# LeeYN-43/Clover

Measured on AMD Instinct MI355X. Metric: video-text pairs/sec (8f x 224^2, 32-tok), full pre-training step, higher is better.
Workload: dtype f16; 1 GPU; VideoSwin-T + BERT-base + 3-layer fusion, MLM + tri-modal exclusive InfoNCE + rank losses, 8f x 224^2, 32-tok; per_gpu_batch=8, global_batch=8, parallelism=dp1

## Files before the change

### clover_amd/_lib.py

```python
import ctypes as C
import os

_HERE = os.path.dirname(os.path.abspath(__file__))
HALF_F16 = os.environ.get('CLOVER_HALF', 'f16').lower() in ('f16', 'fp16', 'float16', 'half')
LIB_PATH = os.environ.get('CLOVER_LIB_PATH') or os.path.join(_HERE, 'libclover_hip_f16.so' if HALF_F16 else 'libclover_hip.so')


_scale_env = os.environ.get('CLOVER_LOSS_SCALE', '1024' if HALF_F16 else '1')
LOSS_SCALE_SPEC = 'dynamic' if _scale_env.strip().lower() == 'dynamic' else float(_scale_env)
LOSS_SCALE = (1024.0 if HALF_F16 else 1.0) if LOSS_SCALE_SPEC == 'dynamic' else LOSS_SCALE_SPEC


def half_dtype():
    import torch
    return torch.float16 if HALF_F16 else torch.bfloat16

ABI_VERSION = 18

ERRORS = {-1: 'CLV_ERR_ARG (bad argument)', -2: 'CLV_ERR_UNSUPPORTED (shape not supported by the kernels)',
          -3: 'CLV_ERR_LAUNCH (HIP launch failed)'}


class ClvAttnGeom(C.Structure):
    _fields_ = [(n, C.c_int32) for n in
                ('mode', 'groups', 'N', 'nH', 'hd', 'D', 'H', 'W', 'wd', 'wh', 'ww', 'sd', 'sh', 'sw',
                 'ldq', 'ldk', 'ldv', 'ldo', 'bwd', 'bwh', 'bww')] + [('scale', C.c_float), ('dropout_p', C.c_float),
                                                                      ('dbias_index', C.c_void_p), ('work', C.c_void_p)]


_p, _i32, _i64, _f = C.c_void_p, C.c_int32, C.c_int64, C.c_float


class ClvFoldEntry(C.Structure):
    _fields_ = [('partial', _p), ('dw', _p), ('db', _p), ('nk', _i64), ('e2', _i64), ('splits', _i32),
                ('sg_shift', _i32), ('block_begin', _i32), ('overwrite', _i32)]


FOLD_MAX = 64


class ClvWgradEntry(C.Structure):
    _fields_ = [('dy', _p), ('x', _p), ('work', _p), ('dw', _p), ('db', _p), ('M', _i64), ('work_floats', _i64),
                ('N', _i32), ('K', _i32),
                ('ldy', _i32), ('ldx', _i32), ('want_bias', _i32), ('splits', _i32), ('overwrite', _i32), ('pad', _i32)]


WGRAD_GROUP_MAX = 80


class ClvDbiasGather(C.Structure):
    _fields_ = [('partial', _p), ('dtable', _p), ('index', _p), ('split_stride', _i64), ('nkt', _i32), ('nH', _i32),
                ('N', _i32), ('nsplit', _i32), ('slot0', _i32), ('nslots', _i32), ('block_begin', _i32), ('pad', _i32)]


DBIAS_GATHER_MAX = 32


class ClvLnReduceEntry(C.Structure):
    _fields_ = [('partial', _p), ('dgamma', _p), ('dbeta', _p), ('nblk', _i32), ('C', _i32), ('block_begin', _i32),
                ('pad', _i32)]


LN_REDUCE_MAX = 64


class ClvLnExtra(C.Structure):
    _fields_ = [('xscale', _p), ('rows_per_sample', _i32), ('drop_p', _f), ('seed', _p), ('dy2', _p), ('dres', _p),
                ('x_is_sum', _i32), ('gather_c', _i32), ('gather_h2', _i32), ('gather_w2', _i32), ('no_reduce', _i32),
                ('q8', _p), ('qscale', _p)]


SIGNATURES = {
    'clv_abi_version': (C.c_int, []),
    'clv_half_type': (C.c_int, []),
    'clv_attn_fwd': (C.c_int, [_p] * 9 + [C.POINTER(ClvAttnGeom), _p]),
    'clv_attn_seq_work_bytes': (C.c_int64, [C.POINTER(ClvAttnGeom)]),
    'clv_attn_seq_max_keys': (C.c_int, []),
    'clv_attn_seq_parts': (C.c_int, [C.POINTER(ClvAttnGeom)]),
    'clv_attn_bwd_work_bytes': (C.c_int64, [C.POINTER(ClvAttnGeom)]),
    'clv_attn_bwd_one_kernel': (C.c_int, [C.POINTER(ClvAttnGeom)]),
    'clv_attn_dbias_index_count': (C.c_int64, [C.POINTER(ClvAttnGeom)]),
    'clv_attn_dbias_index': (C.c_int, [C.POINTER(ClvAttnGeom), _p, _p]),
    'clv_attn_dbias_gather_entry': (C.c_int, [C.POINTER(ClvAttnGeom), _p, _p, C.POINTER(ClvDbiasGather)]),
    'clv_attn_dbias_partial_bytes': (C.c_int64, [_p]),
    'clv_attn_dbias_gather_batch': (C.c_int, [C.POINTER(ClvDbiasGather), _i32, _p]),
    'clv_attn_bwd': (C.c_int, [_p] * 16 + [_i32, C.POINTER(ClvAttnGeom), _p]),
    'clv_softmax_rows_fwd': (C.c_int, [_p] * 5 + [_i64, _i32, _i32, _i32, _f, _f, _p]),
    'clv_softmax_rows_bwd': (C.c_int, [_p] * 4 + [_i64, _i32, _i32, _f, _f, _p]),
    'clv_layernorm_fwd': (C.c_int, [_p] * 8 + [_i64, _i32, _f, _i32, C.POINTER(ClvLnExtra), _p]),
    'clv_layernorm_bwd_blocks': (C.c_int, [_i64, _i32]),
    'clv_layernorm_bwd': (C.c_int, [_p] * 11 + [_i64, _i32, _i32, C.POINTER(ClvLnExtra), _p]),
    'clv_ln_fold_fwd': (C.c_int, [_p] * 6 + [_i32, _i32, _p]),
    'clv_ln_fold_bwd': (C.c_int, [_p] * 9 + [_i32, _i32, _p]),
    'clv_batchnorm1d_fwd': (C.c_int, [_p] * 8 + [_i32, _i32, _f, _f, _i32, _p]),
    'clv_batchnorm1d_bwd': (C.c_int, [_p] * 8 + [_i32, _i32, _i32, _p]),
    'clv_gelu_fwd': (C.c_int, [_p, _p, _i64, _i32, _p]),
    'clv_gelu_bwd': (C.c_int, [_p, _p, _p, _i64, _i32, _p]),
    'clv_patch_embed_fwd': (C.c_int, [_p] * 12 + [_i32] * 7 + [_f, _p]),
    'clv_patch_embed_fwd_fp8': (C.c_int, [_p] * 13 + [_i32] * 7 + [_f, _p]),
    'clv_patch_embed_blend_bwd': (C.c_int, [_p] * 5 + [_i32] * 7 + [_p]),
    'clv_im2col_patches': (C.c_int, [_p, _p, _i32, _i32, _i32, _i32, _p]),
    'clv_linear_wgrad_work_floats': (C.c_int64, [_i64, _i32, _i32]),
    'clv_linear_wgrad': (C.c_int, [_p] * 5 + [_i64, _i32, _i32, _i32, _i32, _p, _p, _i32, _p]),
    'clv_rowgemm_supported': (C.c_int, [_i32, _i32, _i32]),
    'clv_rowgemm': (C.c_int, [_p] * 11 + [_i64, _i32, _i32, _i32, _i32, _i32, _i32, _f, _p]),
    'clv_rowgemm_xs': (C.c_int, [_p] * 11 + [_i64, _i32, _i32, _i32, _i32, _i32, _i32, _f, _p, _i32, _p]),
    'clv_mlp_fused_supported': (C.c_int, [_i32, _i32]),
    'clv_mlp_fused_fwd': (C.c_int, [_p] * 10 + [_i64, _i32, _i32, _f, _p, _i32, _p]),
    'clv_mlp_fused_bwd': (C.c_int, [_p] * 13 + [_i64, _i32, _i32, _p, _i32, _p]),
    'clv_colsum': (C.c_int, [_p, _p, _i64, _i32, _i32, _p]),
    'clv_focal_ce_fwd': (C.c_int, [_p, _i32, _p, _p, _p, _p, _p, _i64, _i32, _f, _p]),
    'clv_focal_ce_bwd': (C.c_int, [_p, _i32, _p, _p, _p, _p, _p, _p, _i64, _i32, _f, _p]),
    'clv_focal_ce_fwd_ld': (C.c_int, [_p, _i32, _p, _p, _p, _p, _p, _i64, _i32, _i64, _f, _p]),
    'clv_focal_ce_bwd_ld': (C.c_int, [_p, _i32, _p, _p, _p, _p, _p, _p, _i64, _i32, _i64, _f, _p]),
    'clv_infonce_work_floats': (C.c_int64, [_i32, _i32]),
    'clv_infonce_fwd': (C.c_int, [_p] * 6 + [_i32, _i32, _i32, _f, _f, _p]),
    'clv_infonce_bwd': (C.c_int, [_p] * 10 + [_i32, _i32, _i32, _f, _f, _p]),
    'clv_infonce_pair_fwd': (C.c_int, [_p] * 4 + [_i32, _i32, _i32, _f, _f, _p]),
    'clv_infonce_pair_bwd': (C.c_int, [_p] * 4 + [_i32, _i32, _i32, _f, _f, _p]),
    'clv_normsoftmax_work_floats': (C.c_int64, [_i32, _i32]),
    'clv_normsoftmax_fwd': (C.c_int, [_p] * 5 + [_i32, _i32, _f, _f, _p]),
    'clv_normsoftmax_bwd': (C.c_int, [_p] * 6 + [_i32, _i32, _f, _p]),
    'clv_infonce_large_min_g': (C.c_int32, []),
    'clv_infonce_fwd_large': (C.c_int, [_p] * 6 + [_i32, _i32, _i32, _f, _f, _p]),
    'clv_infonce_bwd_large': (C.c_int, [_p] * 10 + [_i32, _i32, _i32, _f, _f, _p]),
    'clv_infonce_pair_fwd_large': (C.c_int, [_p] * 4 + [_i32, _i32, _i32, _f, _f, _p]),
    'clv_infonce_pair_bwd_large': (C.c_int, [_p] * 4 + [_i32, _i32, _i32, _f, _f, _p]),
    'clv_normsoftmax_fwd_large': (C.c_int, [_p] * 5 + [_i32, _i32, _f, _f, _p]),
    'clv_normsoftmax_bwd_large': (C.c_int, [_p] * 6 + [_i32, _i32, _f, _p]),
    'clv_sumsq': (C.c_int, [_p, _p, _i64, _p]),
    'clv_adamw_step': (C.c_int, [_p] * 6 + [_i64] + [_f] * 9 + [_p]),
    'clv_gemm_nt_supported': (C.c_int, [_i64, _i32, _i32]),
    'clv_gemm_nt': (C.c_int, [_p] * 6 + [_i64, _i32, _i32, _i64, _i64, _i64, _i32, _p]),
    'clv_gemm_nt_work_bytes': (C.c_int64, [_i64, _i32, _i32]),
    'clv_gemm_nt_ex': (C.c_int, [_p] * 6 + [_i64, _i32, _i32, _i64, _i64, _i64, _i32, _p, _i64, _p]),
    'clv_transpose_batch': (C.c_int, [_p, _p, _p, _i32, _i32, _p]),
    'clv_layernorm_bwd_needs_reduce': (C.c_int, [_i64, _i32]),
    'clv_ln_reduce_batch': (C.c_int, [_p, _i32, _p]),
    'clv_linear_wgrad_in_place': (C.c_int, [C.c_int64, C.c_int32, C.c_int32]),
    'clv_linear_wgrad_class': (C.c_int, [C.c_int64, C.c_int32, C.c_int32]),
    'clv_linear_wgrad_batch_plan': (C.c_int, [_p, _i32]),
    'clv_linear_wgrad_batch': (C.c_int, [_p, _i32, _p]),
    'clv_linear_wgrad_batch_ss': (C.c_int, [_p, _i32, _p, _p]),
    'clv_linear_wgrad_splits': (C.c_int, [_i64, _i32, _i32]),
    'clv_wgrad_fold_batch': (C.c_int, [_p, _i32, _p]),
    'clv_wgrad_fold_batch_ss': (C.c_int, [_p, _i32, _p, _p]),
    'clv_optim_prep_slots': (C.c_int, [_p, _p, _p] + [_f] * 4 + [_p]),
    'clv_sumsq_ranges': (C.c_int, [_p, _p, _i32, _p, _p]),
    'clv_optim_prep': (C.c_int, [_p, _p] + [_f] * 4 + [_p]),
    'clv_adamw_step_dev': (C.c_int, [_p] * 6 + [_i64] + [_f] * 5 + [_p]),
    'clv_ema_update': (C.c_int, [_p, _i32, _i32, C.c_double, _p]),
    'clv_ema_swap': (C.c_int, [_p, _i32, _i32, _p]),
    'clv_grad_report': (C.c_int, [_p, _i32, _p, _i32, _i32, _p, _p, _i32, _p]),
    'clv_quant_fp8_rows': (C.c_int, [_p, _p, _p, _i64, _i32, _i64, _i64, _p]),
    'clv_gemm_nt_fp8_supported': (C.c_int, [_i64, _i32, _i32]),
    'clv_gemm_nt_fp8': (C.c_int, [_p] * 7 + [_i64, _i32, _i32, _i64, _i64, _i64, _i32, _p]),
    'clv_pack_bf16': (C.c_int, [_p, _p, _i64, _p]),
    'clv_sumsq_bf16': (C.c_int, [_p, _p, _i64, _p]),
    'clv_adamw_step_dev_bf16g': (C.c_int, [_p] * 6 + [_i64] + [_f] * 5 + [_p]),
    'clv_sgemm_strided': (C.c_int, [_p] * 4 + [_i64, _i32, _i32, _i64, _i64, _i64, _i64, _i64, _i32, _p]),
    'clv_sgemm_strided_rowsum': (C.c_int, [_p] * 4 + [_i64, _i32, _i32, _i64, _i64, _i64, _i64, _i64, _i32, _p]),
    'clv_sgemm_nt': (C.c_int, [_p] * 4 + [_i64, _i32, _i32, _i64, _i64, _i64, _p]),
    'clv_attn_f32_fwd': (C.c_int, [_p] * 7 + [C.POINTER(ClvAttnGeom), _i32, _p]),
    'clv_attn_f32_bwd_work_floats': (C.c_int64, [C.POINTER(ClvAttnGeom)]),
    'clv_attn_f32_bwd': (C.c_int, [_p] * 12 + [C.POINTER(ClvAttnGeom), _p]),
    'clv_qa_answer_rows': (C.c_int, [_p, _i32, _i32, _i32, _i32, _i32, _i64, _p, _p, _p]),
    'clv_qa_head_supported': (C.c_int, [_i32, _i32, _i32]),
    'clv_qa_head_fwd': (C.c_int, [_p] * 9 + [_f, _f] + [_p] * 5 + [_i32] * 4 + [_p]),
    'clv_qa_mc_ce_fwd': (C.c_int, [_p] * 4 + [_i32, _i32, _p]),
# ... 44 lines not shown
```

### clover_amd/backbones/swin_transformer_3d.py

```python
from functools import lru_cache

import numpy as np
import torch
import torch.nn as nn
import torch.nn.functional as F
import torch.utils.checkpoint as _checkpoint

from .. import ops
from ..builder import BACKBONES
from ..nn import GELU, DropPath, LayerNorm, Linear, trunc_normal_

BF16 = ops.BF16


def get_window_size(x_size, window_size, shift_size=None):
    use_ws = list(window_size)
    use_ss = list(shift_size) if shift_size is not None else None
    for i in range(len(x_size)):
        if x_size[i] <= window_size[i]:
            use_ws[i] = x_size[i]
            if use_ss is not None:
                use_ss[i] = 0
    if shift_size is None:
        return tuple(use_ws)
    return tuple(use_ws), tuple(use_ss)


def build_relative_position_index(window_size):
    wd, wh, ww = window_size
    coords = torch.stack(torch.meshgrid(torch.arange(wd), torch.arange(wh), torch.arange(ww), indexing='ij'))
    cf = torch.flatten(coords, 1)
    rel = (cf[:, :, None] - cf[:, None, :]).permute(1, 2, 0).contiguous()
    rel[:, :, 0] += wd - 1
    rel[:, :, 1] += wh - 1
    rel[:, :, 2] += ww - 1
    rel[:, :, 0] *= (2 * wh - 1) * (2 * ww - 1)
    rel[:, :, 1] *= (2 * ww - 1)
    return rel.sum(-1)


def region_id_windows(Dp, Hp, Wp, window_size, shift_size):
    img = np.zeros((Dp, Hp, Wp), dtype=np.int32)
    cnt = 0
    ws, ss = window_size, shift_size
    for d in (slice(-ws[0]), slice(-ws[0], -ss[0]), slice(-ss[0], None)):
        for h in (slice(-ws[1]), slice(-ws[1], -ss[1]), slice(-ss[1], None)):
            for w in (slice(-ws[2]), slice(-ws[2], -ss[2]), slice(-ss[2], None)):
                img[d, h, w] = cnt
                cnt += 1
    x = img.reshape(Dp // ws[0], ws[0], Hp // ws[1], ws[1], Wp // ws[2], ws[2])
    return np.ascontiguousarray(x.transpose(0, 2, 4, 1, 3, 5).reshape(-1, ws[0] * ws[1] * ws[2]))


@lru_cache(maxsize=64)
def _window_geometry_cached(x_size, cfg_ws, cfg_ss, device_str):
    ws, ss = get_window_size(x_size, cfg_ws, cfg_ss)
    padded = tuple(int(np.ceil(x_size[i] / ws[i])) * ws[i] for i in range(3))
    rid = None
    if any(s > 0 for s in ss):
        rid = torch.from_numpy(region_id_windows(padded[0], padded[1], padded[2], ws, ss)).to(device_str)
    return ws, ss, rid, padded


def window_geometry(x_size, cfg_ws, cfg_ss, device):
    ws, ss, rid, _ = _window_geometry_cached(tuple(x_size), tuple(cfg_ws), tuple(cfg_ss), str(device))
    return ws, ss, rid


def gathered_bias(table, rel_index, N):
    nH = table.shape[1]
    return table.float()[rel_index[:N, :N].reshape(-1)].view(N, N, nH).permute(2, 0, 1).contiguous()


def mask_blend_weight(mask, T, H, W):
    _, _, mh, mw = mask.shape
    w = mask.unsqueeze(-1).unsqueeze(-3).expand(-1, T, -1, H // mh, -1, W // mw)
    return w.flatten(2, 3).flatten(3, 4).unsqueeze(1)


class Mlp(nn.Module):
    def __init__(self, in_features, hidden_features=None, out_features=None, act_layer=GELU, drop=0.):
        super().__init__()
        out_features = out_features or in_features
        hidden_features = hidden_features or in_features
        self.fc1 = Linear(in_features, hidden_features)
        self.act = act_layer()
        self.fc2 = Linear(hidden_features, out_features)
        self.drop = nn.Dropout(drop)
        for lin in (self.fc1, self.fc2):
            lin.weight._clv_want_t = ops.wants_transposed(lin.out_features, lin.in_features)
        if ops.mlp_fused_shape(in_features, hidden_features) and out_features == in_features:
            self.fc2.weight._clv_want_t = True

    def forward(self, x):
        if (type(self.act) is GELU and self.drop.p == 0.0 and self.fc1.bias is not None
                and ops.mlp_gelu_ok(x, self.fc1.out_features)):
            return ops.mlp_gelu(x, self.fc1.weight, self.fc1.bias, self.fc2.weight, self.fc2.bias)
        return self.drop(self.fc2(self.drop(self.act(self.fc1(x)))))


class WindowAttention3D(nn.Module):

    def __init__(self, dim, window_size, num_heads, qkv_bias=False, qk_scale=None, attn_drop=0., proj_drop=0.):
        super().__init__()
        self.dim = dim
        self.window_size = window_size
        self.num_heads = num_heads
        head_dim = dim // num_heads
        self.scale = qk_scale or head_dim ** -0.5
        if qk_scale is not None and abs(qk_scale - head_dim ** -0.5) > 1e-12:
            raise NotImplementedError('qk_scale override is not supported by the HIP attention kernel')
        if attn_drop != 0.:
            raise NotImplementedError('attn_drop_rate > 0 is not supported (Clover configs use 0)')
        self.relative_position_bias_table = nn.Parameter(
            torch.zeros((2 * window_size[0] - 1) * (2 * window_size[1] - 1) * (2 * window_size[2] - 1), num_heads))
        self.register_buffer('relative_position_index', build_relative_position_index(window_size))
        self.qkv = Linear(dim, dim * 3, bias=qkv_bias)
        self.proj = Linear(dim, dim)
        for lin in (self.qkv, self.proj):
            lin.weight._clv_want_t = ops.wants_transposed(lin.out_features, lin.in_features)
        self.proj_drop = nn.Dropout(proj_drop)
        trunc_normal_(self.relative_position_bias_table, std=.02)

    def forward(self, x, ws, ss, rid):
        N = ws[0] * ws[1] * ws[2]
        qkv = self.qkv(x)
        o = ops.window_attention(qkv, self.relative_position_bias_table, rid if any(s > 0 for s in ss) else None,
                                 ws, ss, self.num_heads, table_window=self.window_size)
        return self.proj_drop(self.proj(o))


class SwinTransformerBlock3D(nn.Module):
    def __init__(self, dim, num_heads, window_size=(2, 7, 7), shift_size=(0, 0, 0), mlp_ratio=4., qkv_bias=True,
                 qk_scale=None, drop=0., attn_drop=0., drop_path=0., act_layer=GELU, norm_layer=LayerNorm,
                 use_checkpoint=False):
        super().__init__()
        self.dim, self.num_heads = dim, num_heads
        self.window_size, self.shift_size = window_size, shift_size
        self.mlp_ratio = mlp_ratio
        self.use_checkpoint = use_checkpoint
        for i in range(3):
            assert 0 <= shift_size[i] < window_size[i], 'shift_size must in 0-window_size'
        self.norm1 = norm_layer(dim)
        self.attn = WindowAttention3D(dim, window_size=window_size, num_heads=num_heads, qkv_bias=qkv_bias,
                                      qk_scale=qk_scale, attn_drop=attn_drop, proj_drop=drop)
        self.drop_path = DropPath(drop_path) if drop_path > 0. else nn.Identity()
        self.norm2 = norm_layer(dim)
        self.mlp = Mlp(in_features=dim, hidden_features=int(dim * mlp_ratio), act_layer=act_layer, drop=drop)

    def attn_part(self, x):
        B, D, H, W, C = x.shape
        ws, ss, rid = window_geometry((D, H, W), self.window_size, self.shift_size, x.device)
        pad_d1 = (ws[0] - D % ws[0]) % ws[0]
        pad_b = (ws[1] - H % ws[1]) % ws[1]
        pad_r = (ws[2] - W % ws[2]) % ws[2]
        if pad_d1 or pad_b or pad_r:
            x = F.pad(x, (0, 0, 0, pad_r, 0, pad_b, 0, pad_d1))
        x = self.attn(x, ws, ss, rid)
        if pad_d1 or pad_b or pad_r:
            x = x[:, :D, :H, :W, :].contiguous()
        return x

    def forward_part1(self, x):
        return self.attn_part(self.norm1(x))

    def forward_part2(self, x):
        return self.drop_path(self.mlp(self.norm2(x)))

    def _dp_scale(self, x):
        return self.drop_path.scale(x) if isinstance(self.drop_path, DropPath) else None

    def forward_pending(self, x, branch=None, bscale=None):
        if self._fused_ok(x):
            return self._forward_pending_fused(x, DropPath.apply_scale(branch, bscale) if branch is not None else None)
        if branch is None:
            y1, s0 = self.norm1(x, return_sum=True)
        else:
            y1, s0 = self.norm1(branch, residual=x, return_sum=True, x_scale=bscale)
        a = self.attn_part(y1)
        y2, s1 = self.norm2(a, residual=s0, return_sum=True, x_scale=self._dp_scale(a))
        m = self.mlp(y2)
        return s1, m, self._dp_scale(m)

    def _fused_ok(self, x):
        B, D, H, W, C = x.shape
        ws = get_window_size((D, H, W), self.window_size)
        no_pad = D % ws[0] == 0 and H % ws[1] == 0 and W % ws[2] == 0
        return (x.is_cuda and no_pad and self.mlp.drop.p == 0.0 and self.attn.proj_drop.p == 0.0
                and self.attn.qkv.bias is not None and type(self.mlp.act) is GELU
                and ops.fused_block_supported(C, self.mlp.fc1.out_features))

    def _forward_pending_fused(self, x, branch):
        B, D, H, W, C = x.shape
        ws, ss, rid = window_geometry((D, H, W), self.window_size, self.shift_size, x.device)
        at = self.attn
        if branch is None:
            qkv, s0 = ops.ln_linear(x, None, self.norm1.weight, self.norm1.bias, at.qkv.weight, at.qkv.bias,
                                    self.norm1.eps, stream_out=True)
        else:
            qkv, s0 = ops.ln_linear(branch, x, self.norm1.weight, self.norm1.bias, at.qkv.weight, at.qkv.bias,
                                    self.norm1.eps)
        o = ops.window_attention(qkv, at.relative_position_bias_table, rid if any(s > 0 for s in ss) else None, ws, ss,
                                 self.num_heads, table_window=at.window_size)
        a = at.proj(o)
        m, s1 = ops.fused_mlp(a, s0, self.norm2.weight, self.norm2.bias, self.mlp.fc1.weight, self.mlp.fc1.bias,
                              self.mlp.fc2.weight, self.mlp.fc2.bias, self.norm2.eps, x_scale=self._dp_scale(a))
        return s1, m, self._dp_scale(m)

    def forward(self, x, mask_matrix=None):
        s, m, sc = self.forward_pending(x)
        return s + DropPath.apply_scale(m, sc)


class PatchMerging(nn.Module):
    def __init__(self, dim, norm_layer=LayerNorm):
        super().__init__()
        self.dim = dim
        self.reduction = Linear(4 * dim, 2 * dim, bias=False)
        self.reduction.weight._clv_want_t = ops.wants_transposed(2 * dim, 4 * dim)
        self.norm = norm_layer(4 * dim)

    @staticmethod
    def merge_gather(x):
        B, D, H, W, C = x.shape
        if (H % 2 == 1) or (W % 2 == 1):
            x = F.pad(x, (0, 0, 0, W % 2, 0, H % 2))
        B, D, H, W, C = x.shape
        v = x.view(B, D, H // 2, 2, W // 2, 2, C).permute(0, 1, 2, 4, 5, 3, 6)
        return v.reshape(B, D, H // 2, W // 2, 4 * C)

    def forward(self, x):
        return self.reduction(self.norm(self.merge_gather(x)))

    def forward_pending(self, s, m, sc):
        B, D, H, W, C = s.shape
        if ops.parity.enabled():
            return self.forward(ops.parity.rnd('stream', s + DropPath.apply_scale(m, sc)))
        if not s.is_cuda or H % 2 or W % 2 or C % 8 or not isinstance(self.norm, LayerNorm):
            return self.forward(s + DropPath.apply_scale(m, sc))
        y = ops.merge_layer_norm(m, self.norm.weight, self.norm.bias, self.norm.eps, residual=s, x_scale=sc)
        return self.reduction(y)


class BasicLayer(nn.Module):
    def __init__(self, dim, depth, num_heads, window_size=(1, 7, 7), mlp_ratio=4., qkv_bias=False, qk_scale=None,
                 drop=0., attn_drop=0., drop_path=0., norm_layer=LayerNorm, downsample=None, use_checkpoint=False):
        super().__init__()
        self.window_size = window_size
        self.shift_size = tuple(i // 2 for i in window_size)
        self.depth = depth
        self.use_checkpoint = use_checkpoint
        self.blocks = nn.ModuleList([
            SwinTransformerBlock3D(dim=dim, num_heads=num_heads, window_size=window_size,
                                   shift_size=(0, 0, 0) if (i % 2 == 0) else self.shift_size, mlp_ratio=mlp_ratio,
                                   qkv_bias=qkv_bias, qk_scale=qk_scale, drop=drop, attn_drop=attn_drop,
                                   drop_path=drop_path[i] if isinstance(drop_path, list) else drop_path,
                                   norm_layer=norm_layer, use_checkpoint=use_checkpoint)
            for i in range(depth)])
        self.downsample = downsample(dim=dim, norm_layer=norm_layer) if downsample is not None else None

    def forward(self, x):
        s, m, sc = self.forward_pending(x)
        if self.downsample is not None and hasattr(self.downsample, 'forward_pending'):
            return self.downsample.forward_pending(s, m, sc)
        x = s + DropPath.apply_scale(m, sc)
        if self.downsample is not None:
            x = self.downsample(x)
        return x

    def forward_pending(self, x, branch=None, bscale=None):
        for blk in self.blocks:
            if self.use_checkpoint and torch.is_grad_enabled():
                draws = blk.mlp.drop.p > 0 or blk.attn.proj_drop.p > 0
                x, branch, bscale = _checkpoint.checkpoint(blk.forward_pending, x, branch, bscale, use_reentrant=False,
                                                           preserve_rng_state=draws)
            else:
                x, branch, bscale = blk.forward_pending(x, branch, bscale)
        return x, branch, bscale


class PatchEmbed3D(nn.Module):
    def __init__(self, patch_size=(2, 4, 4), in_chans=3, embed_dim=96, norm_layer=None, stride=(2, 4, 4)):
        super().__init__()
        if tuple(patch_size) != (2, 4, 4) or tuple(stride) != (2, 4, 4) or in_chans != 3:
            raise NotImplementedError('the HIP patch-embed kernel covers patch=stride=(2,4,4), in_chans=3 '
                                      '(every Clover / VideoSwin config)')
        self.patch_size = tuple(patch_size)
        self.in_chans = in_chans
        self.embed_dim = embed_dim
        self.proj = nn.Conv3d(in_chans, embed_dim, kernel_size=patch_size, stride=stride)
        self.norm = norm_layer(embed_dim) if norm_layer is not None else None

    def pad(self, x):
        _, _, D, H, W = x.size()
        if W % self.patch_size[2] != 0:
            x = F.pad(x, (0, self.patch_size[2] - W % self.patch_size[2]))
        if H % self.patch_size[1] != 0:
            x = F.pad(x, (0, 0, 0, self.patch_size[1] - H % self.patch_size[1]))
        if D % self.patch_size[0] != 0:
            x = F.pad(x, (0, 0, 0, 0, 0, self.patch_size[0] - D % self.patch_size[0]))
        return x

    def tokens(self, x, mask_token=None, vmask=None, want_clean=True):
        x = self.pad(x)
        g, b = (self.norm.weight, self.norm.bias) if self.norm is not None else (None, None)
        eps = self.norm.eps if self.norm is not None else 1e-5
        return ops.patch_embed(x, self.proj.weight, self.proj.bias, g, b, mask_token, vmask, want_clean, eps)

    def tokens_stacked(self, x, mask_token, vmask):
        x = self.pad(x)
        g, b = (self.norm.weight, self.norm.bias) if self.norm is not None else (None, None)
        eps = self.norm.eps if self.norm is not None else 1e-5
        return ops.patch_embed_stacked(x, self.proj.weight, self.proj.bias, g, b, mask_token, vmask, eps)

    def forward(self, x):
        clean, _ = self.tokens(x)
        return clean.permute(0, 4, 1, 2, 3)


@BACKBONES.register_module()
class SwinTransformer3D(nn.Module):
    def __init__(self, pretrained=None, pretrained2d=True, patch_size=(2, 4, 4), stride=(2, 4, 4), in_chans=3,
                 embed_dim=96, depths=[2, 2, 6, 2], num_heads=[3, 6, 12, 24], window_size=(8, 7, 7), mlp_ratio=4.,
                 qkv_bias=True, qk_scale=None, drop_rate=0., attn_drop_rate=0., drop_path_rate=0.1,
                 norm_layer=LayerNorm, patch_norm=True, frozen_stages=-1, use_checkpoint=False, mask_token=False):
        super().__init__()
        if norm_layer is nn.LayerNorm:
            norm_layer = LayerNorm
        self.pretrained = pretrained
        self.pretrained2d = pretrained2d
        self.num_layers = len(depths)
        self.embed_dim = embed_dim
        self.patch_norm = patch_norm
        self.frozen_stages = frozen_stages
        self.window_size = tuple(window_size)
        self.patch_size = tuple(patch_size)
        self.fp16_enabled = False
        self.patch_embed = PatchEmbed3D(patch_size=patch_size, in_chans=in_chans, embed_dim=embed_dim, stride=stride,
                                        norm_layer=norm_layer if self.patch_norm else None)
        self.pos_drop = nn.Dropout(p=drop_rate)
        dpr = [x.item() for x in torch.linspace(0, drop_path_rate, sum(depths))]
        self.layers = nn.ModuleList()
        for i_layer in range(self.num_layers):
            self.layers.append(BasicLayer(
                dim=int(embed_dim * 2 ** i_layer), depth=depths[i_layer], num_heads=num_heads[i_layer],
                window_size=self.window_size, mlp_ratio=mlp_ratio, qkv_bias=qkv_bias, qk_scale=qk_scale,
                drop=drop_rate, attn_drop=attn_drop_rate,
                drop_path=dpr[sum(depths[:i_layer]):sum(depths[:i_layer + 1])], norm_layer=norm_layer,
                downsample=PatchMerging if i_layer < self.num_layers - 1 else None, use_checkpoint=use_checkpoint))
        self.num_features = int(embed_dim * 2 ** (self.num_layers - 1))
        self.norm = norm_layer(self.num_features)
        if mask_token:
            self.mask_token = nn.Parameter(torch.zeros(1, self.embed_dim, 1, 1, 1))
            trunc_normal_(self.mask_token, mean=0., std=.02)
        self._freeze_stages()

    def _freeze_stages(self):
        if self.frozen_stages >= 0:
            self.patch_embed.eval()
            for p in self.patch_embed.parameters():
                p.requires_grad = False
        if self.frozen_stages >= 1:
            self.pos_drop.eval()
            for i in range(0, self.frozen_stages):
                m = self.layers[i]
                m.eval()
                for p in m.parameters():
                    p.requires_grad = False

    def inflate_state_dict(self, state_dict):
        sd = {k: v for k, v in state_dict.items() if 'relative_position_index' not in k and 'attn_mask' not in k}
        w = sd['patch_embed.proj.weight']
        sd['patch_embed.proj.weight'] = w.unsqueeze(2).repeat(1, 1, self.patch_size[0], 1, 1) / self.patch_size[0]
        own = self.state_dict()
        for k in [k for k in sd if 'relative_position_bias_table' in k]:
            pre = sd[k]
            L1, nH1 = pre.size()
            nH2 = own[k].size(1)
            L2 = (2 * self.window_size[1] - 1) * (2 * self.window_size[2] - 1)
            wd = self.window_size[0]
            if nH1 == nH2 and L1 != L2:
                S1 = int(L1 ** 0.5)
                pre = F.interpolate(pre.permute(1, 0).view(1, nH1, S1, S1),
                                    size=(2 * self.window_size[1] - 1, 2 * self.window_size[2] - 1), mode='bicubic')
                pre = pre.view(nH2, L2).permute(1, 0)
            sd[k] = pre.repeat(2 * wd - 1, 1)
        return sd

    def inflate_weights(self, state_dict):
        sd = self.inflate_state_dict(state_dict)
        own = self.state_dict()
        bad = [k for k, v in sd.items() if k in own and tuple(own[k].shape) != tuple(v.shape)]
        res = self.load_state_dict({k: v for k, v in sd.items() if k not in bad}, strict=False)
        return list(res.missing_keys), list(res.unexpected_keys), bad

    def init_weights(self, pretrained=None):
        def _init_weights(m):
            if isinstance(m, nn.Linear):
                trunc_normal_(m.weight, std=.02)
                if m.bias is not None:
                    nn.init.constant_(m.bias, 0)
            elif isinstance(m, nn.LayerNorm):
                nn.init.constant_(m.bias, 0)
                nn.init.constant_(m.weight, 1.0)
        if pretrained:
            self.pretrained = pretrained
        if isinstance(self.pretrained, str):
            self.apply(_init_weights)
            ckpt = torch.load(self.pretrained, map_location='cpu')
            sd = ckpt.get('state_dict', ckpt)
            if self.pretrained2d:
                self.inflate_weights(sd)
            else:
                sd = {(k[len('backbone.'):] if k.startswith('backbone.') else k): v for k, v in sd.items()}
                self.load_state_dict(sd, strict=False)
        elif self.pretrained is None:
            self.apply(_init_weights)
        else:
            raise TypeError('pretrained must be a str or None')

    def _draw_drop_paths(self, B, device):
        if not self.training:
            return
        if getattr(self, '_dp_mods', None) is None:
            self._dp_mods = [m for m in self.modules() if isinstance(m, DropPath) and m.drop_prob > 0]
            self._dp_tables = {}
        if not self._dp_mods:
            return
        key = (str(device), int(B))
        tab = self._dp_tables.get(key)
        if tab is None:
            keep = torch.tensor([1.0 - m.drop_prob for m in self._dp_mods], device=device)[:, None]
            tab = self._dp_tables[key] = (keep.expand(len(self._dp_mods), B).contiguous(), 1.0 / keep)
        scales = torch.bernoulli(tab[0]) * tab[1]
        for i, m in enumerate(self._dp_mods):
            m.preset(scales[i])

    CUT_STAGE = 2

    def late_parameters(self):
        if self.CUT_STAGE >= self.num_layers - 1:
            return []
        mods = list(self.layers[self.CUT_STAGE:]) + [self.norm]
        return [q for m in mods for q in m.parameters()]

    def _stages(self, x, mid_cut=None):
        self._draw_drop_paths(x.shape[0], x.device)
        x = self.pos_drop(x)
        for i, layer in enumerate(self.layers[:-1]):
            if mid_cut is not None and i == self.CUT_STAGE:
                leaf = x.detach().requires_grad_()
                mid_cut.append((x, leaf))
                x = leaf
            x = layer(x)
        s, m, sc = self.layers[-1].forward_pending(x)
        return self.norm(m, residual=s, x_scale=sc)

    def forward_tokens(self, x, mask=None, mid_cut=None):
        if mask is None:
            t, _ = self.patch_embed.tokens(x)
        else:
            _, t = self.patch_embed.tokens(x, self.mask_token, mask, want_clean=False)
        return self._stages(t, mid_cut)

    def forward_pair(self, x, mask):
        B = x.shape[0]
        clean, masked = self.patch_embed.tokens(x, self.mask_token, mask)
        y = self._stages(torch.cat([clean, masked], dim=0))
        return y[:B], y[B:]

    def forward_both(self, x, mask, mid_cut=None):
        return self._stages(self.patch_embed.tokens_stacked(x, self.mask_token, mask), mid_cut)

    def forward(self, x, mask=None):
        y = self.forward_tokens(x, mask).permute(0, 4, 1, 2, 3)
        if mask is not None:
            _, _, T, H, W = (x.shape[0], 0, (x.shape[2] + 1) // 2, (x.shape[3] + 3) // 4, (x.shape[4] + 3) // 4)
            w = mask_blend_weight(mask, T, H, W).type_as(y)
            return y, w
        return y

    def train(self, mode=True):
        super().train(mode)
        self._freeze_stages()
```

### clover_amd/csrc/attention.hip

```cpp
#include "common.hpp"
#include <type_traits>
#include "../../include/clover_hip.h"

namespace {

constexpr int WAVES = 4;
constexpr int THREADS = WAVES * 64;
constexpr int DKV_THREADS(int nkt) { return nkt >= 13 ? 512 : THREADS; }

constexpr int DBIAS_GROUPS_PER_SLICE = 64;
constexpr int DBIAS_CHUNK_MB = 128;
constexpr int DBIAS_HEADS_PER_WAVE = 4;

struct Geom {
    ClvAttnGeom g;
    int nWh, nWw, nW;
    unsigned drop_thresh;
    float inv_keep;
    int ts_d, ts_h, tcst, tlen, tls;
    int tb0, tbn;
    int tsplit;
    int grp0;
    int nparts, pt16;
    int lddq, lddk, lddv;
// ... 23 lines not shown
    const int ty = tr / G.g.ww, tx = tr - ty * G.g.ww;
    int d = wz * G.g.wd + tz + G.g.sd; if (d >= G.g.D) d -= G.g.D;
    int h = wy * G.g.wh + ty + G.g.sh; if (h >= G.g.H) h -= G.g.H;
    int w = wx * G.g.ww + tx + G.g.sw; if (w >= G.g.W) w -= G.g.W;
    return (((int64_t)b * G.g.D + d) * G.g.H + h) * G.g.W + w;
}

__device__ __forceinline__ float4 table_bias4(const char* tp, const int* kb_ptr) {
    const int4 kb = *reinterpret_cast<const int4*>(kb_ptr);
    float4 b;
    b.x = *reinterpret_cast<const float*>(tp - kb.x);
    b.y = *reinterpret_cast<const float*>(tp - kb.y);
    b.z = *reinterpret_cast<const float*>(tp - kb.z);
    b.w = *reinterpret_cast<const float*>(tp - kb.w);
    return b;
}

__device__ __forceinline__ int xcd_remap(int bid, int nblk) {
    const int q = nblk >> 3, r = nblk & 7, xcd = bid & 7, idx = bid >> 3;
    return (xcd < r ? xcd * (q + 1) : r * (q + 1) + (xcd - r) * q) + idx;
}

template <int HD>
__device__ __forceinline__ void load_frags(Frag8 (&f)[(HD + 31) / 32], const bf16_t* rowp, bool valid, int lane) {
    constexpr int KS = (HD + 31) / 32;
#pragma unroll
    for (int s = 0; s < KS; ++s) {
        const int hd0 = s * 32 + (lane >> 4) * 8;
        if (valid && hd0 < HD) f[s].u4 = *reinterpret_cast<const uint4*>(rowp + hd0);
        else f[s].u4 = make_uint4(0, 0, 0, 0);
    }
}

template <int HD>
__device__ __forceinline__ void lds_frags(Frag8 (&f)[(HD + 31) / 32], const bf16_t* rowp, int lane) {
    constexpr int KS = (HD + 31) / 32;
#pragma unroll
    for (int s = 0; s < KS; ++s) {
        const int hd0 = s * 32 + (lane >> 4) * 8;
        if (hd0 < HD) f[s].u4 = *reinterpret_cast<const uint4*>(rowp + hd0);
        else f[s].u4 = make_uint4(0, 0, 0, 0);
    }
}

template <int HD, int NK, bool SCALE = false>
__device__ __forceinline__ void stage(const int* row_s, const bf16_t* base, int ld, int h, int N, bf16_t* rm, int tid,
                                      int nthr = THREADS, float mul = 1.f) {
    constexpr int CH = HD / 8, LDR = HD + 8;
    for (int idx = tid; idx < NK * CH; idx += nthr) {
        const int n = idx / CH, c = idx - n * CH;
        uint4 val = make_uint4(0, 0, 0, 0);
        if (n < N) val = *reinterpret_cast<const uint4*>(base + (int64_t)row_s[n] * ld + h * HD + c * 8);
        if (SCALE) {
            uint32_t* w = reinterpret_cast<uint32_t*>(&val);
#pragma unroll
            for (int e = 0; e < 4; ++e)
                w[e] = pack2bf(half_lo(w[e]) * mul, half_hi(w[e]) * mul);
        }
        *reinterpret_cast<uint4*>(rm + n * LDR + c * 8) = val;
    }
}

template <int NK>
__device__ __forceinline__ void token_rows(const Geom& G, int grp, int* row_s, int tid, int nthr = THREADS, int s0 = 0) {
    for (int n = tid; n < NK; n += nthr) row_s[n] = (s0 + n < G.g.N) ? (int)tok_row(G, grp, s0 + n) : 0;
    __syncthreads();
}
__device__ __forceinline__ int64_t loop_row(const Geom& G, const int* row_s, int grp, int n) {
    return G.nparts > 1 ? (int64_t)grp * G.g.N + n : (int64_t)row_s[n];
}

typedef short v4s_t __attribute__((ext_vector_type(4)));
__device__ __forceinline__ uint2 tr4(const bf16_t* base, int LD, int row0, int c0, int lr) {
    const bf16_t* p = base + (row0 + (lr >> 2)) * LD + c0 + (lr & 3) * 4;
    const v4s_t r = __builtin_amdgcn_ds_read_tr16_b64_v4i16((__attribute__((address_space(3))) v4s_t*)p);
    union { v4s_t v; uint2 u; } cv;
    cv.v = r;
    return cv.u;
}

constexpr float LOG2E = 1.4426950408889634f;
__device__ __forceinline__ float exp_sub(float x, float negL2) { return __builtin_amdgcn_exp2f(fmaf(x, LOG2E, negL2)); }

template <int HD, int NKT, bool DROP, int MODE>
__global__ void __launch_bounds__(THREADS, (NKT <= 16 ? 3 : 1)) attn_fwd_kernel(
    const bf16_t* __restrict__ q, const bf16_t* __restrict__ k, const bf16_t* __restrict__ v,
    bf16_t* __restrict__ o, float* __restrict__ lse, const float* __restrict__ bias,
    const int* __restrict__ rid, const float* __restrict__ kmask, const unsigned long long* __restrict__ seedp,
    Geom G) {
    constexpr int NK = NKT * 16, KS = (HD + 31) / 32, LDR = HD + 8, NC = HD / 16;
    extern __shared__ __attribute__((aligned(16))) unsigned char smem[];
    bf16_t* Ks = reinterpret_cast<bf16_t*>(smem);
    bf16_t* Vs = Ks + NK * LDR;
    float* aux = reinterpret_cast<float*>(Vs + NK * LDR);

    const int tid = threadIdx.x, lane = tid & 63, wave = tid >> 6;
    const int bid = xcd_remap(blockIdx.x, gridDim.x);
    const int part = bid % G.tsplit;
    const int sp = (bid / G.tsplit) % G.nparts, gh = bid / (G.tsplit * G.nparts);
    const int grp = gh / G.g.nH, h = gh - grp * G.g.nH;
    const int N = G.g.N;
    const int s0 = sp * G.pt16, Ns = min(N - s0, G.pt16);

    int* row_s = reinterpret_cast<int*>(aux + (MODE == 1 ? 1 : 2) * NK);
    int* linb_s = row_s + NK;
    float* tab_s = reinterpret_cast<float*>(linb_s + NK);
    int* flag_s = reinterpret_cast<int*>(tab_s + G.tls);
    if (tid == 0) *flag_s = 0;
    token_rows<NK>(G, grp, row_s, tid, THREADS, s0);
    constexpr int PRE = NKT <= 16 ? (NKT + WAVES - 1) / WAVES : 1;
    const int nqt = (N + 15) >> 4;
    Frag8 qpre[PRE][KS];
    if (PRE > 1) {
#pragma unroll
        for (int ti = 0; ti < PRE; ++ti) {
            const int qt = wave + WAVES * part + ti * WAVES * G.tsplit;
            const int nq = qt * 16 + (lane & 15);
            const bool qv = qt < nqt && nq < N;
            load_frags<HD>(qpre[ti], q + loop_row(G, row_s, grp, qv ? nq : 0) * G.g.ldq + h * HD, qv, lane);
        }
    }
    stage<HD, NK, true>(row_s, k, G.g.ldk, h, Ns, Ks, tid, THREADS, G.g.scale * LOG2E);
    stage<HD, NK>(row_s, v, G.g.ldv, h, Ns, Vs, tid);
    if (MODE == 1 && bias) load_bias_table<NK>(G, bias, h, tab_s, linb_s, tid, THREADS, LOG2E);
    int* rid_s = reinterpret_cast<int*>(aux);
    float* kadd = aux + NK;
    const int wloc = (G.g.mode == 1) ? grp % G.nW : 0;
    int differs = 0;
    for (int n = tid; n < NK; n += THREADS) {
        if (MODE == 1 && rid) {
            const int rv = (n < N) ? rid[wloc * N + n] : 0;
            rid_s[n] = rv;
            if (n < N) differs |= rv != rid[wloc * N];
        }
        if (MODE == 0) kadd[n] = (n < Ns) ? (kmask ? kmask[(int64_t)grp * N + s0 + n] * LOG2E : 0.f) : -INFINITY;
    }
    if (differs) *flag_s = 1;
    __syncthreads();
    const bool masked = *flag_s != 0;

    const int lg = lane >> 4, lr = lane & 15;
    Frag8 onesf;
    onesf.u[0] = onesf.u[1] = onesf.u[2] = onesf.u[3] = CLV_ONE_PAIR;
    constexpr int UNR = PRE > 1 ? PRE : 1;
#pragma unroll UNR
    for (int ti = 0; ti < (NKT + WAVES - 1) / WAVES; ++ti) {
        const int qt = wave + WAVES * part + ti * WAVES * G.tsplit;
        if (qt >= nqt) break;
        const int nq = qt * 16 + lr;
        const bool qv = nq < N;
        const int64_t qrow = loop_row(G, row_s, grp, qv ? nq : 0);
        Frag8 qf[KS];
        if (PRE > 1) {
#pragma unroll
            for (int s = 0; s < KS; ++s) qf[s] = qpre[PRE > 1 ? ti : 0][s];
        } else {
            load_frags<HD>(qf, q + qrow * G.g.ldq + h * HD, qv, lane);
        }

        constexpr int CH = NKT > 16 ? 14 : NKT;
        float p[CH][4];
        const bool tb = MODE == 1 && bias != nullptr;
        const char* tp = reinterpret_cast<const char*>(tab_s) + (tb ? linb_s[qv ? nq : 0] + 4 * G.tcst : 0);
        const int rq = (MODE == 1 && rid && qv) ? rid_s[nq] : 0;
        float4 bnext = make_float4(0.f, 0.f, 0.f, 0.f);
        if (tb) bnext = table_bias4(tp, linb_s + lg * 4);
        f32x4_t oacc[NC];
        f32x4_t sacc = {0.f, 0.f, 0.f, 0.f};
#pragma unroll
        for (int c = 0; c < NC; ++c) oacc[c] = (f32x4_t){0.f, 0.f, 0.f, 0.f};
        float m = -INFINITY, sum = 0.f;
#pragma unroll
        for (int c0 = 0; c0 < NKT; c0 += CH) {
            constexpr int dummy = 0; (void)dummy;
            const int ct = (NKT - c0) < CH ? (NKT - c0) : CH;
            float mc = -INFINITY;
#pragma unroll
            for (int tt = 0; tt < CH; ++tt) {
                if (tt >= ct) break;
                const int t = c0 + tt;
                Frag8 kf[KS];
                lds_frags<HD>(kf, Ks + (t * 16 + lr) * LDR, lane);
                const int key0 = t * 16 + lg * 4;
                asm volatile("" ::: "memory");
                const float4 bv = bnext;
                if (tb && t + 1 < NKT) bnext = table_bias4(tp, linb_s + (t + 1) * 16 + lg * 4);
                f32x4_t acc = {bv.x, bv.y, bv.z, bv.w};
                if (MODE == 0) {
                    const float4 ka = *reinterpret_cast<const float4*>(kadd + key0);
                    acc[0] += ka.x; acc[1] += ka.y; acc[2] += ka.z; acc[3] += ka.w;
                } else if ((t + 1) * 16 > Ns) {
#pragma unroll
                    for (int r = 0; r < 4; ++r) acc[r] = (key0 + r < Ns) ? acc[r] : -INFINITY;
                }
                if (masked) {
                    const int4 rk = *reinterpret_cast<const int4*>(rid_s + key0);
                    acc[0] += (rk.x != rq) ? -100.0f * LOG2E : 0.0f;
                    acc[1] += (rk.y != rq) ? -100.0f * LOG2E : 0.0f;
                    acc[2] += (rk.z != rq) ? -100.0f * LOG2E : 0.0f;
                    acc[3] += (rk.w != rq) ? -100.0f * LOG2E : 0.0f;
                }
#pragma unroll
                for (int s = 0; s < KS; ++s) acc = mfma16(kf[s], qf[s], acc);
#pragma unroll
                for (int r = 0; r < 4; ++r) {
                    p[tt][r] = acc[r];
                    mc = fmaxf(mc, acc[r]);
                }
            }
            mc = grp4_max(mc);
            if (CH < NKT) {
                const float mn = fmaxf(m, mc);
                const float sc = (m == -INFINITY) ? 0.f : __builtin_amdgcn_exp2f(m - mn);
                if (c0 > 0) {
#pragma unroll
                    for (int c = 0; c < NC; ++c)
#pragma unroll
                        for (int r = 0; r < 4; ++r) oacc[c][r] *= sc;
#pragma unroll
                    for (int r = 0; r < 4; ++r) sacc[r] *= sc;
                    sum *= sc;
                }
                m = mn;
            } else {
                m = mc;
            }
            float csum = 0.f;
#pragma unroll
            for (int tt = 0; tt < CH; ++tt) {
                if (tt >= ct) break;
#pragma unroll
                for (int r = 0; r < 4; ++r) {
                    const float e = __builtin_amdgcn_exp2f(p[tt][r] - m);
                    p[tt][r] = e;
                    if (DROP) csum += e;
                }
            }
            if (DROP) {
                sum += grp4_sum(csum);
                const unsigned long long sd = *seedp;
                const unsigned rowid = (unsigned)((grp * G.g.nH + h) * N + nq);
#pragma unroll
                for (int tt = 0; tt < CH; ++tt) {
                    if (tt >= ct) break;
#pragma unroll
                    for (int r = 0; r < 4; ++r)
                        p[tt][r] *= keep_scale(sd, rowid, (unsigned)(s0 + (c0 + tt) * 16 + lg * 4 + r), G.drop_thresh, G.inv_keep);
                }
            }
#pragma unroll
            for (int s2 = 0; s2 < (CH + 1) / 2; ++s2) {
                if (2 * s2 >= ct) break;
                const bool tail = 2 * s2 + 1 >= ct;
                Frag8 pf;
                pf.u[0] = pack2bf(p[2 * s2][0], p[2 * s2][1]);
                pf.u[1] = pack2bf(p[2 * s2][2], p[2 * s2][3]);
                pf.u[2] = tail ? 0u : pack2bf(p[tail ? 0 : 2 * s2 + 1][0], p[tail ? 0 : 2 * s2 + 1][1]);
                pf.u[3] = tail ? 0u : pack2bf(p[tail ? 0 : 2 * s2 + 1][2], p[tail ? 0 : 2 * s2 + 1][3]);
                const int kt = c0 + 2 * s2;
#pragma unroll
                for (int c = 0; c < NC; ++c) {
                    Frag8 vf;
                    vf.u2[0] = tr4(Vs, LDR, kt * 16 + lg * 4, c * 16, lr);
                    vf.u2[1] = tail ? make_uint2(0u, 0u) : tr4(Vs, LDR, (kt + 1) * 16 + lg * 4, c * 16, lr);
                    oacc[c] = mfma16(vf, pf, oacc[c]);
                }
                if (!DROP) sacc = mfma16(onesf, pf, sacc);
            }
        }
        if (!DROP) sum = sacc[0];
        if (qv && lg == 0) lse[sp * G.lse_ps + ((int64_t)grp * G.g.nH + h) * N + nq] = (m + __log2f(sum)) * (1.0f / LOG2E);
        const float inv = 1.0f / sum;
        if (qv) {
            bf16_t* orow = o + sp * G.o_ps + qrow * G.g.ldo + h * HD + lg * 4;
#pragma unroll
            for (int c = 0; c < NC; ++c) {
                uint2 w;
                w.x = pack2bf(oacc[c][0] * inv, oacc[c][1] * inv);
                w.y = pack2bf(oacc[c][2] * inv, oacc[c][3] * inv);
                *reinterpret_cast<uint2*>(orow + c * 16) = w;
            }
        }
    }
}

template <int HD, int NKT, bool DROP, int MODE>
__global__ void __launch_bounds__(DKV_THREADS(NKT), (NKT > 16 ? 2 : ((NKT == 13 || NKT == 14) && HD == 32 && MODE == 1 ? 6 : 1))) attn_bwd_dq_kernel(
    const bf16_t* __restrict__ q, const bf16_t* __restrict__ k, const bf16_t* __restrict__ v,
    const bf16_t* __restrict__ o, const bf16_t* __restrict__ dout, const float* __restrict__ lse,
    const float* __restrict__ bias, const int* __restrict__ rid, const float* __restrict__ kmask,
    bf16_t* __restrict__ dq, bf16_t* __restrict__ ds_out, float* __restrict__ dsum,
    const unsigned long long* __restrict__ seedp, Geom G) {
    constexpr int NK = NKT * 16, KS = (HD + 31) / 32, LDR = HD + 8, NC = HD / 16;
    extern __shared__ __attribute__((aligned(16))) unsigned char smem[];
    bf16_t* Ks = reinterpret_cast<bf16_t*>(smem);
    bf16_t* Vs = Ks + NK * LDR;
    float* aux = reinterpret_cast<float*>(Vs + NK * LDR);
    int* rid_s = reinterpret_cast<int*>(aux);
    float* kadd = aux + NK;
    int* row_s = reinterpret_cast<int*>(aux + 2 * NK);
    int* linb_s = row_s + NK;
    float* tab_s = reinterpret_cast<float*>(linb_s + NK);

    const int tid = threadIdx.x, lane = tid & 63, wave = tid >> 6, nthr = blockDim.x, nwaves = nthr >> 6;
    const int bid = xcd_remap(blockIdx.x, gridDim.x);
    const int part = bid % G.tsplit;
    const int sp = (bid / G.tsplit) % G.nparts, gh = bid / (G.tsplit * G.nparts);
    const int grp = gh / G.g.nH + G.grp0, h = gh % G.g.nH;
    const int N = G.g.N;
    const int s0 = sp * G.pt16, Ns = min(N - s0, G.pt16);
    const bool tb = MODE == 1 && bias != nullptr;
    int* flag_s = reinterpret_cast<int*>(tab_s + G.tls);
    if (tid == 0) *flag_s = 0;

    token_rows<NK>(G, grp, row_s, tid, nthr, s0);
    constexpr int NWAVES = DKV_THREADS(NKT) / 64;
    constexpr int PRE = (NKT + NWAVES - 1) / NWAVES;
    constexpr bool PREF = NKT <= 16;
    const int nqt = (N + 15) >> 4;
    Frag8 qpre[PREF ? PRE : 1][KS], dopre[PREF ? PRE : 1][KS], opre[PREF ? PRE : 1][KS];
    if (PREF) {
#pragma unroll
        for (int ti = 0; ti < PRE; ++ti) {
            const int qt = wave + nwaves * part + ti * nwaves * G.tsplit;
            const int nq = qt * 16 + (lane & 15);
            const bool qv = qt < nqt && nq < N;
            const int64_t qrow = loop_row(G, row_s, grp, qv ? nq : 0);
            load_frags<HD>(qpre[ti], q + qrow * G.g.ldq + h * HD, qv, lane);
            load_frags<HD>(dopre[ti], dout + qrow * G.g.ldo + h * HD, qv, lane);
            load_frags<HD>(opre[ti], o + qrow * G.g.ldo + h * HD, qv, lane);
        }
    }
    stage<HD, NK, true>(row_s, k, G.g.ldk, h, Ns, Ks, tid, nthr, G.g.scale * LOG2E);
    stage<HD, NK>(row_s, v, G.g.ldv, h, Ns, Vs, tid, nthr);
    if (tb) load_bias_table<NK>(G, bias, h, tab_s, linb_s, tid, nthr, LOG2E);
    const int wloc = (G.g.mode == 1) ? grp % G.nW : 0;
    int differs = 0;
    for (int n = tid; n < NK; n += nthr) {
        if (MODE == 1 && rid) {
            const int rv = (n < N) ? rid[wloc * N + n] : 0;
            rid_s[n] = rv;
// ... 221 lines not shown
                    bv.z = *reinterpret_cast<const float*>(tp + qb.z);
                    bv.w = *reinterpret_cast<const float*>(tp + qb.w);
                }
                f32x4_t sacc = {bv.x, bv.y, bv.z, bv.w}, pacc = {0.f, 0.f, 0.f, 0.f};
                if (masked) {
                    const int4 rq4 = *reinterpret_cast<const int4*>(rid_s + qn0);
                    sacc[0] += (rq4.x != rk) ? -100.0f * LOG2E : 0.0f;
                    sacc[1] += (rq4.y != rk) ? -100.0f * LOG2E : 0.0f;
                    sacc[2] += (rq4.z != rk) ? -100.0f * LOG2E : 0.0f;
                    sacc[3] += (rq4.w != rk) ? -100.0f * LOG2E : 0.0f;
                }
                Frag8 qf[KS], dof[KS];
                lds_frags<HD>(qf, Qs + (qt * 16 + lr) * LDR, lane);
                lds_frags<HD>(dof, dOs + (qt * 16 + lr) * LDR, lane);
#pragma unroll
                for (int s = 0; s < KS; ++s) {
                    sacc = mfma16(qf[s], kf[s], sacc);
                    pacc = mfma16(dof[s], vf[s], pacc);
                }
                const float4 L4 = *reinterpret_cast<const float4*>(L_s + qn0);
                const float4 D4 = *reinterpret_cast<const float4*>(D_s + qn0);
                const float Lr[4] = {L4.x, L4.y, L4.z, L4.w}, Dr[4] = {D4.x, D4.y, D4.z, D4.w};
#pragma unroll
                for (int r = 0; r < 4; ++r) {
                    const float pr = __builtin_amdgcn_exp2f(sacc[r] + Lr[r]);
                    float ks = 1.f;
                    if (DROP)
                        ks = keep_scale(sd, (unsigned)((grp * G.g.nH + h) * N + s0 + qn0 + r), (unsigned)nk, G.drop_thresh,
                                        G.inv_keep);
                    pv[r] = pr * ks;
                    dsv[r] = pr * (pacc[r] * ks - Dr[r]);
                }
                pf.u[half * 2 + 0] = pack2bf(pv[0], pv[1]);
                pf.u[half * 2 + 1] = pack2bf(pv[2], pv[3]);
                dsf.u[half * 2 + 0] = pack2bf(dsv[0], dsv[1]);
                dsf.u[half * 2 + 1] = pack2bf(dsv[2], dsv[3]);
            }
#pragma unroll
            for (int c = 0; c < NC; ++c) {
                Frag8 a;
                const bool tail = (NKT & 1) && 2 * qp + 1 >= NKT;
                a.u2[0] = tr4(dOs, LDR, (2 * qp) * 16 + lg * 4, c * 16, lr);
                a.u2[1] = tail ? make_uint2(0u, 0u) : tr4(dOs, LDR, (2 * qp + 1) * 16 + lg * 4, c * 16, lr);
                dvacc[c] = mfma16(a, pf, dvacc[c]);
                a.u2[0] = tr4(Qs, LDR, (2 * qp) * 16 + lg * 4, c * 16, lr);
                a.u2[1] = tail ? make_uint2(0u, 0u) : tr4(Qs, LDR, (2 * qp + 1) * 16 + lg * 4, c * 16, lr);
                dkacc[c] = mfma16(a, dsf, dkacc[c]);
            }
        }
        if (kv) {
            bf16_t* dvrow = dv + sp * G.dv_ps + krow * G.lddv + h * HD + lg * 4;
            bf16_t* dkrow = dk + sp * G.dk_ps + krow * G.lddk + h * HD + lg * 4;
#pragma unroll
            for (int c = 0; c < NC; ++c) {
                uint2 w;
                w.x = pack2bf(dvacc[c][0], dvacc[c][1]);
                w.y = pack2bf(dvacc[c][2], dvacc[c][3]);
                *reinterpret_cast<uint2*>(dvrow + c * 16) = w;
                w.x = pack2bf(dkacc[c][0] * (1.0f / LOG2E), dkacc[c][1] * (1.0f / LOG2E));
                w.y = pack2bf(dkacc[c][2] * (1.0f / LOG2E), dkacc[c][3] * (1.0f / LOG2E));
                *reinterpret_cast<uint2*>(dkrow + c * 16) = w;
            }
        }
    }
}

#ifndef ONE_MINW
#define ONE_MINW 4
#endif
#ifndef ONE_ABL
#define ONE_ABL 0
#endif
constexpr int ONE_CWAVES(int nkt) { return (nkt + 1) / 2; }
constexpr int ONE_SWAVES(int nkt) { return nkt > 16 ? 2 : 1; }
constexpr int ONE_LDR(int hd, int nkt) { return nkt > 16 ? hd : hd + 8; }
template <int HD, int NKT>
size_t one_lds(int tls) {
    return 2 * (size_t)(NKT * 16) * ONE_LDR(HD, NKT) * 2 + 5 * (size_t)NKT * 16 * 4 + (size_t)tls * 4 + 16 +
           2 * (size_t)ONE_CWAVES(NKT) * 4 * 256 * 2 + (NKT > 16 ? (size_t)NKT * 16 * HD * 2 : 0);
}

__device__ __forceinline__ void lds_barrier() { asm volatile("s_waitcnt lgkmcnt(0)\n\ts_barrier" ::: "memory"); }

template <int HD, int NKT>
__global__ void __launch_bounds__((ONE_CWAVES(NKT) + ONE_SWAVES(NKT)) * 64, ONE_MINW) attn_bwd_one_kernel(
    const bf16_t* __restrict__ q, const bf16_t* __restrict__ k, const bf16_t* __restrict__ v,
    const bf16_t* __restrict__ o, const bf16_t* __restrict__ dout, const float* __restrict__ lse,
    const float* __restrict__ bias, const int* __restrict__ rid, bf16_t* __restrict__ dq, bf16_t* __restrict__ dk,
    bf16_t* __restrict__ dv, bf16_t* __restrict__ ds_out, float* __restrict__ trace, Geom G) {
    constexpr int NK = NKT * 16, KS = (HD + 31) / 32, LDR = ONE_LDR(HD, NKT), NC = HD / 16, CH = HD / 8;
    constexpr int NWC = ONE_CWAVES(NKT), NS = ONE_SWAVES(NKT), NTHR = (NWC + NS) * 64, NQP = (NKT + 1) / 2;
    constexpr bool KREG = NKT <= 16;
#ifdef ONE_TRACE
    const unsigned long long t_start = __builtin_amdgcn_s_memtime();
#define ONE_T(i) if (trace && (threadIdx.x & 63) == 0) trace[(int64_t)blockIdx.x * 16 + (i)] = (float)(__builtin_amdgcn_s_memtime() - t_start)
#define ONE_TV(i, v) if (trace && (threadIdx.x & 63) == 0) trace[(int64_t)blockIdx.x * 16 + (i)] = (float)(v)
    unsigned long long bw_s = 0, bw_c = 0;
#define ONE_BAR(acc) { const unsigned long long t0_ = __builtin_amdgcn_s_memtime(); lds_barrier(); acc += __builtin_amdgcn_s_memtime() - t0_; }
#else
#define ONE_T(i)
#define ONE_TV(i, v)
#define ONE_BAR(acc) lds_barrier()
#endif
    constexpr int TW = 4 * 256;
    static_assert(KS == 1 && CH == 4, "one-kernel backward: HD = 32");
    extern __shared__ __attribute__((aligned(16))) unsigned char smem[];
    bf16_t* Qs = reinterpret_cast<bf16_t*>(smem);
    bf16_t* dOs = Qs + NK * LDR;
    float* L_s = reinterpret_cast<float*>(dOs + NK * LDR);
    float* D_s = L_s + NK;
    int* row_s = reinterpret_cast<int*>(D_s + NK);
    int* linb_s = row_s + NK;
    int* rid_s = linb_s + NK;
    float* tab_s = reinterpret_cast<float*>(rid_s + NK);
    int* flag_s = reinterpret_cast<int*>(tab_s + G.tls);
    bf16_t* T_s = reinterpret_cast<bf16_t*>(flag_s + 4);

    const int tid = threadIdx.x, lane = tid & 63, wave = tid >> 6, lg = lane >> 4, lr = lane & 15;
    const int gh = xcd_remap(blockIdx.x, gridDim.x);
    const int grp = gh / G.g.nH + G.grp0, h = gh % G.g.nH;
    const int N = G.g.N;
    constexpr int nt = NKT;
    const bool tb = bias != nullptr;
    if (tid == 0) *flag_s = 0;
    token_rows<NK>(G, grp, row_s, tid, NTHR);
    if (wave == 0) { ONE_T(0); }

    Frag8 kf[2], vf[2];
    float kmv[2];
    if (wave < NWC) {
#pragma unroll
        for (int ti = 0; ti < 2; ++ti) {
            const int nk = (wave * 2 + ti) * 16 + lr;
            const bool kv = nk < N;
            const int64_t krow = row_s[kv ? nk : 0];
            Frag8 t1[KS], t2[KS];
            load_frags<HD>(t1, k + krow * G.g.ldk + h * HD, kv, lane);
            load_frags<HD>(t2, v + krow * G.g.ldv + h * HD, kv, lane);
            kf[ti] = t1[0];
            vf[ti] = t2[0];
            kmv[ti] = kv ? 0.f : -INFINITY;
        }
    }
    static_assert(!KREG || (size_t)NK * HD <= (size_t)NWC * TW, "K rows fit one T buffer");
    bf16_t* Kst = T_s + (KREG ? 1 : 2) * NWC * TW;
    {
        const float qmul = G.g.scale * LOG2E;
        constexpr int NP = (NK * CH + NTHR - 1) / NTHR;
        constexpr int NTAB = 3;
        uint4 vq[NP], vd[NP], vo[NP], vk[NP];
#pragma unroll
        for (int j = 0; j < NP; ++j) {
            const int idx = tid + j * NTHR, n = idx / CH, c = idx - n * CH;
            vq[j] = vd[j] = vo[j] = vk[j] = make_uint4(0, 0, 0, 0);
            if (idx < NK * CH && n < N) {
                const int64_t r = row_s[n];
                vq[j] = *reinterpret_cast<const uint4*>(q + r * G.g.ldq + h * HD + c * 8);
                vd[j] = *reinterpret_cast<const uint4*>(dout + r * G.g.ldo + h * HD + c * 8);
                vo[j] = *reinterpret_cast<const uint4*>(o + r * G.g.ldo + h * HD + c * 8);
                vk[j] = *reinterpret_cast<const uint4*>(k + r * G.g.ldk + h * HD + c * 8);
            }
        }
        static_assert(NK <= NTHR, "one token per thread");
        const int wloc = grp % G.nW;
        const float lv = (tid < N) ? lse[((int64_t)grp * G.g.nH + h) * N + tid] : 0.f;
        const int rv = (rid && tid < N) ? rid[wloc * N + tid] : 0, rv0 = rid ? rid[wloc * N] : 0;
        float tv[NTAB];
#pragma unroll
        for (int j = 0; j < NTAB; ++j) {
            const int i = tid + j * NTHR;
            tv[j] = i < G.tbn ? bias[(int64_t)(G.tb0 + i) * G.g.nH + h] : 0.f;
        }
#pragma unroll
        for (int j = 0; j < NP; ++j) {
            const int idx = tid + j * NTHR, n = idx / CH, c = idx - n * CH;
            auto sc2 = [&](uint32_t w) { return pack2bf(half_lo(w) * qmul, half_hi(w) * qmul); };
            auto dot2 = [](uint32_t a, uint32_t b) {
                return half_lo(a) * half_lo(b) + half_hi(a) * half_hi(b);
            };
            float d = (dot2(vd[j].x, vo[j].x) + dot2(vd[j].y, vo[j].y)) + (dot2(vd[j].z, vo[j].z) + dot2(vd[j].w, vo[j].w));
            d += __shfl_xor(d, 1, 64);
            d += __shfl_xor(d, 2, 64);
            if (idx < NK * CH) {
                *reinterpret_cast<uint4*>(Qs + n * LDR + c * 8) = make_uint4(sc2(vq[j].x), sc2(vq[j].y), sc2(vq[j].z), sc2(vq[j].w));
                *reinterpret_cast<uint4*>(dOs + n * LDR + c * 8) = vd[j];
                *reinterpret_cast<uint4*>(Kst + n * HD + c * 8) = vk[j];
                if (c == 0) D_s[n] = d;
            }
        }
        if (tid < NK) {
            L_s[tid] = (tid < N) ? -lv * LOG2E : -INFINITY;
            linb_s[tid] = (tid < N) ? 4 * win_lin(G, tid) : 0;
            if (rid) {
                rid_s[tid] = rv;
                if (tid < N && rv != rv0) *flag_s = 1;
            }
        }
#pragma unroll
        for (int j = 0; j < NTAB; ++j) {
            const int i = tid + j * NTHR;
            if (i < G.tbn) tab_s[i] = tv[j] * LOG2E;
        }
    }
    if (wave == 0) { ONE_T(1); }
    lds_barrier();
    if (wave == 0) { ONE_T(2); }

    if (wave >= NWC) {
        auto kt_frag = [&](int jp, int c) {
            Frag8 f;
            f.u2[0] = tr4(Kst, HD, (2 * jp) * 16 + lg * 4, c * 16, lr);
            f.u2[1] = (2 * jp + 1 < NKT) ? tr4(Kst, HD, (2 * jp + 1) * 16 + lg * 4, c * 16, lr) : make_uint2(0u, 0u);
            return f;
        };
        Frag8 ktf[KREG ? NWC : 1][NC];
        if (KREG) {
#pragma unroll
            for (int jp = 0; jp < NWC; ++jp)
#pragma unroll
                for (int c = 0; c < NC; ++c) ktf[KREG ? jp : 0][c] = kt_frag(jp, c);
        }
        const int sw = wave - NWC;
        bf16_t* dsbase = (tb && ds_out) ? ds_out + (((int64_t)(grp - G.grp0) * G.g.nH + h) * nt * NKT * 64 + lane) * 4 : nullptr;
        auto dq_chunk = [&](int pc, int bt) {
            const bf16_t* Tb = T_s + bt * (NWC * TW);
#pragma unroll
            for (int half = 0; half < 2; ++half) {
                const int qt = 2 * pc + half;
                if (qt >= NKT) break;
                if (NS == 2 && half != sw) continue;
                Frag8 bq[NWC];
#pragma unroll
                for (int jp = 0; jp < NWC; ++jp) {
                    bq[jp].u2[0] = tr4(Tb + jp * TW + (half * 2 + 0) * 256, 16, lg * 4, 0, lr);
                    bq[jp].u2[1] = (2 * jp + 1 < NKT) ? tr4(Tb + jp * TW + (half * 2 + 1) * 256, 16, lg * 4, 0, lr) : make_uint2(0u, 0u);
                }
                if (!(ONE_ABL & 1) && dsbase) {
                    bf16_t* dsq = dsbase + (int64_t)qt * NKT * 256;
#pragma unroll
                    for (int kt = 0; kt < NKT; ++kt) *reinterpret_cast<uint2*>(dsq + kt * 256) = bq[kt >> 1].u2[kt & 1];
                }
                f32x4_t qacc[NC];
#pragma unroll
                for (int c = 0; c < NC; ++c) qacc[c] = (f32x4_t){0.f, 0.f, 0.f, 0.f};
#pragma unroll
                for (int jp = 0; jp < NWC; ++jp)
#pragma unroll
                    for (int c = 0; c < NC; ++c)
                        qacc[c] = mfma16(KREG ? ktf[KREG ? jp : 0][c] : kt_frag(jp, c), bq[jp], qacc[c]);
                const int qn = qt * 16 + lr;
                if (qn < N) {
                    bf16_t* drow = dq + (int64_t)row_s[qn] * G.lddq + h * HD + lg * 4;
#pragma unroll
                    for (int c = 0; c < NC; ++c) {
                        uint2 w2;
                        w2.x = pack2bf(qacc[c][0] * G.g.scale, qacc[c][1] * G.g.scale);
                        w2.y = pack2bf(qacc[c][2] * G.g.scale, qacc[c][3] * G.g.scale);
                        *reinterpret_cast<uint2*>(drow + c * 16) = w2;
                    }
                }
            }
        };
#pragma unroll 1
        for (int p = 0; p < NQP; ++p) {
            if (!(ONE_ABL & 2) && p > 0) dq_chunk(p - 1, (p - 1) & 1);
            ONE_BAR(bw_s);
        }
        ONE_T(5);
        ONE_TV(8, bw_s);
        if (!(ONE_ABL & 2)) dq_chunk(NQP - 1, (NQP - 1) & 1);
        ONE_T(6);
        return;
    }

    int ko[2], rk[2];
    f32x4_t dvacc[2][NC], dkacc[2][NC];
#pragma unroll
    for (int ti = 0; ti < 2; ++ti) {
#pragma unroll
        for (int c = 0; c < NC; ++c) {
            dvacc[ti][c] = (f32x4_t){0.f, 0.f, 0.f, 0.f};
            dkacc[ti][c] = (f32x4_t){0.f, 0.f, 0.f, 0.f};
        }
        const int nk = (wave * 2 + ti) * 16 + lr;
        rk[ti] = (rid && nk < N) ? rid_s[nk] : 0;
        ko[ti] = linb_s[nk < N ? nk : 0] - 4 * G.tcst;
    }
    const bool masked = rid && *flag_s != 0;

    auto chunk = [&](int p, auto nh_c, auto masked_c) {
        constexpr int NH = decltype(nh_c)::value;
        constexpr bool MASKED = decltype(masked_c)::value;
        const bf16_t* Qb = Qs + p * 32 * LDR;
        const bf16_t* dOb = dOs + p * 32 * LDR;
        bf16_t* Tw = T_s + ((p & 1) * NWC + wave) * TW;
        Frag8 pf[2], dsf[2];
#pragma unroll
        for (int ti = 0; ti < 2; ++ti) pf[ti].u4 = dsf[ti].u4 = make_uint4(0, 0, 0, 0);
#pragma unroll
        for (int half = 0; half < NH; ++half) {
            const int qn0 = (2 * p + half) * 16 + lg * 4;
            Frag8 qf, dof;
            qf.u4 = *reinterpret_cast<const uint4*>(Qb + (half * 16 + lr) * LDR + lg * 8);
            dof.u4 = *reinterpret_cast<const uint4*>(dOb + (half * 16 + lr) * LDR + lg * 8);
            const float4 L4 = *reinterpret_cast<const float4*>(L_s + qn0);
            const float4 D4 = *reinterpret_cast<const float4*>(D_s + qn0);
            const float Lr[4] = {L4.x, L4.y, L4.z, L4.w}, Dr[4] = {D4.x, D4.y, D4.z, D4.w};
            const int4 qb = *reinterpret_cast<const int4*>(linb_s + qn0);
            int4 rq4 = make_int4(0, 0, 0, 0);
            if (MASKED) rq4 = *reinterpret_cast<const int4*>(rid_s + qn0);
#pragma unroll
            for (int ti = 0; ti < 2; ++ti) {
                f32x4_t sacc, pacc = {0.f, 0.f, 0.f, 0.f};
                if (!(ONE_ABL & 16)) {
                    const char* tp = reinterpret_cast<const char*>(tab_s) - ko[ti];
                    sacc[0] = kmv[ti] + *reinterpret_cast<const float*>(tp + qb.x);
                    sacc[1] = kmv[ti] + *reinterpret_cast<const float*>(tp + qb.y);
                    sacc[2] = kmv[ti] + *reinterpret_cast<const float*>(tp + qb.z);
                    sacc[3] = kmv[ti] + *reinterpret_cast<const float*>(tp + qb.w);
                } else {
                    sacc = (f32x4_t){kmv[ti], kmv[ti], kmv[ti], kmv[ti]};
                }
                if (MASKED) {
                    sacc[0] += (rq4.x != rk[ti]) ? -100.0f * LOG2E : 0.0f;
                    sacc[1] += (rq4.y != rk[ti]) ? -100.0f * LOG2E : 0.0f;
                    sacc[2] += (rq4.z != rk[ti]) ? -100.0f * LOG2E : 0.0f;
                    sacc[3] += (rq4.w != rk[ti]) ? -100.0f * LOG2E : 0.0f;
                }
                sacc = mfma16(qf, kf[ti], sacc);
                pacc = mfma16(dof, vf[ti], pacc);
                float pv[4], dsv[4];
#pragma unroll
                for (int r = 0; r < 4; ++r) {
                    pv[r] = (ONE_ABL & 32) ? sacc[r] + Lr[r] : __builtin_amdgcn_exp2f(sacc[r] + Lr[r]);
                    dsv[r] = pv[r] * (pacc[r] - Dr[r]);
                }
                pf[ti].u[half * 2 + 0] = pack2bf(pv[0], pv[1]);
                pf[ti].u[half * 2 + 1] = pack2bf(pv[2], pv[3]);
                dsf[ti].u[half * 2 + 0] = pack2bf(dsv[0], dsv[1]);
                dsf[ti].u[half * 2 + 1] = pack2bf(dsv[2], dsv[3]);
                if (!(ONE_ABL & 4))
                *reinterpret_cast<uint2*>(Tw + (half * 2 + ti) * 256 + lr * 16 + lg * 4) =
                    make_uint2(dsf[ti].u[half * 2 + 0], dsf[ti].u[half * 2 + 1]);
            }
        }
#pragma unroll
        for (int c = 0; c < ((ONE_ABL & 8) ? 0 : NC); ++c) {
            Frag8 ad, aq;
            ad.u2[0] = tr4(dOb, LDR, lg * 4, c * 16, lr);
            ad.u2[1] = NH == 2 ? tr4(dOb, LDR, 16 + lg * 4, c * 16, lr) : make_uint2(0u, 0u);
            aq.u2[0] = tr4(Qb, LDR, lg * 4, c * 16, lr);
            aq.u2[1] = NH == 2 ? tr4(Qb, LDR, 16 + lg * 4, c * 16, lr) : make_uint2(0u, 0u);
#pragma unroll
            for (int ti = 0; ti < 2; ++ti) {
                dvacc[ti][c] = mfma16(ad, pf[ti], dvacc[ti][c]);
                dkacc[ti][c] = mfma16(aq, dsf[ti], dkacc[ti][c]);
            }
        }
    };
    auto loop = [&](auto masked_c) {
#pragma unroll 1
        for (int p = 0; p < NKT / 2; ++p) {
            chunk(p, std::integral_constant<int, 2>{}, masked_c);
            ONE_BAR(bw_c);
        }
        if (NKT & 1) {
            chunk(NKT / 2, std::integral_constant<int, 1>{}, masked_c);
            ONE_BAR(bw_c);
        }
    };
    if (masked) loop(std::true_type{});
    else loop(std::false_type{});
    if (wave == 0) { ONE_T(3); ONE_TV(7, bw_c); }
    if (wave == NWC - 1) { ONE_TV(9, bw_c); }
#pragma unroll
    for (int ti = 0; ti < 2; ++ti) {
        const int nk = (wave * 2 + ti) * 16 + lr;
        if (nk < N) {
            const int64_t krow = row_s[nk];
            bf16_t* dvrow = dv + krow * G.lddv + h * HD + lg * 4;
            bf16_t* dkrow = dk + krow * G.lddk + h * HD + lg * 4;
#pragma unroll
            for (int c = 0; c < NC; ++c) {
                uint2 w;
                w.x = pack2bf(dvacc[ti][c][0], dvacc[ti][c][1]);
                w.y = pack2bf(dvacc[ti][c][2], dvacc[ti][c][3]);
                *reinterpret_cast<uint2*>(dvrow + c * 16) = w;
                w.x = pack2bf(dkacc[ti][c][0] * (1.0f / LOG2E), dkacc[ti][c][1] * (1.0f / LOG2E));
                w.y = pack2bf(dkacc[ti][c][2] * (1.0f / LOG2E), dkacc[ti][c][3] * (1.0f / LOG2E));
                *reinterpret_cast<uint2*>(dkrow + c * 16) = w;
            }
        }
    }
    if (wave == 0) { ONE_T(4); }
}

__global__ void __launch_bounds__(256) dbias_sum_kernel(const bf16_t* __restrict__ ds, float4* __restrict__ partial,
                                                        int groups, int64_t E2) {
    const int64_t e = (int64_t)blockIdx.x * blockDim.x + threadIdx.x;
    if (e >= E2) return;
    float acc[8];
#pragma unroll
    for (int i = 0; i < 8; ++i) acc[i] = 0.f;
    int g = blockIdx.y;
    const int gs = gridDim.y;
    for (; g + 3 * gs < groups; g += 4 * gs) {
        Frag8 v0, v1, v2, v3;
        v0.u4 = *reinterpret_cast<const uint4*>(ds + ((int64_t)g * E2 + e) * 8);
        v1.u4 = *reinterpret_cast<const uint4*>(ds + ((int64_t)(g + gs) * E2 + e) * 8);
        v2.u4 = *reinterpret_cast<const uint4*>(ds + ((int64_t)(g + 2 * gs) * E2 + e) * 8);
        v3.u4 = *reinterpret_cast<const uint4*>(ds + ((int64_t)(g + 3 * gs) * E2 + e) * 8);
#pragma unroll
        for (int i = 0; i < 8; ++i) acc[i] += (bf2f(v0.h[i]) + bf2f(v1.h[i])) + (bf2f(v2.h[i]) + bf2f(v3.h[i]));
    }
    for (; g < groups; g += gs) {
        Frag8 v;
        v.u4 = *reinterpret_cast<const uint4*>(ds + ((int64_t)g * E2 + e) * 8);
#pragma unroll
        for (int i = 0; i < 8; ++i) acc[i] += bf2f(v.h[i]);
    }
    float4* out = partial + ((int64_t)blockIdx.y * E2 + e) * 2;
    out[0] = make_float4(acc[0], acc[1], acc[2], acc[3]);
    out[1] = make_float4(acc[4], acc[5], acc[6], acc[7]);
}

__device__ __forceinline__ void dbias_gather_wave(const float* __restrict__ dense, float* __restrict__ dtable, int nkt,
// ... 55 lines not shown
    float a = 0.f;
    for (int kb = lane; kb < NK; kb += 64) {
        const int off = trow[kb];
        if (off < 0) continue;
        const float* pe = dh + off;
        int sp = 0;
        for (; sp + 4 <= nsplit; sp += 4)
            a += (pe[sp * split_stride] + pe[(sp + 1) * split_stride]) + (pe[(sp + 2) * split_stride] + pe[(sp + 3) * split_stride]);
        for (; sp < nsplit; ++sp) a += pe[sp * split_stride];
    }
    a = wave_sum(a);
    if (lane == 0) dtable[w] += a;
}

struct GatherTable {
    ClvDbiasGather e[CLV_DBIAS_GATHER_MAX];
    int n;
};
__global__ void __launch_bounds__(256) dbias_split_sum_batch_kernel(GatherTable tab) {
    int idx = 0;
    for (int i = 1; i < tab.n; ++i)
        if ((int)blockIdx.x >= tab.e[i].block_begin) idx = i;
    const ClvDbiasGather& en = tab.e[idx];
    const int64_t n4 = en.split_stride >> 2;
    const int64_t i4 = ((int64_t)((int)blockIdx.x - en.block_begin)) * 256 + threadIdx.x;
    if (i4 >= n4 || en.nsplit <= 1) return;
    float4* base = static_cast<float4*>(const_cast<void*>(en.partial));
    float4 a = base[i4];
    for (int sp = 1; sp < en.nsplit; ++sp) {
        const float4 b = base[i4 + sp * n4];
        a.x += b.x; a.y += b.y; a.z += b.z; a.w += b.w;
    }
    base[i4] = a;
}

__global__ void __launch_bounds__(256) dbias_gather_batch_kernel(GatherTable tab) {
    int idx = 0;
    for (int i = 1; i < tab.n; ++i)
        if ((int)blockIdx.x >= tab.e[i].block_begin) idx = i;
    const ClvDbiasGather& en = tab.e[idx];
    const int hg = en.pad > 0 ? en.pad : 1, ngrp = en.nH / hg;
    const int wl = ((int)blockIdx.x - en.block_begin) * 4 + (threadIdx.x >> 6), lane = threadIdx.x & 63;
    if (wl >= en.nslots * ngrp) return;
    const int slot = en.slot0 + wl / ngrp, h0 = (wl % ngrp) * hg;
    const int NK = en.nkt * 16, nqt = (en.N + 15) >> 4;
    const int64_t hstride = (int64_t)nqt * en.nkt * 256;
    const float* dh = static_cast<const float*>(en.partial) + h0 * hstride;
    const int* trow = static_cast<const int*>(en.index) + slot * NK;
    const int nsplit = en.nsplit;
    const int64_t split_stride = en.split_stride;
    float a[4] = {0.f, 0.f, 0.f, 0.f};
    for (int kb0 = lane; kb0 < NK; kb0 += 256) {
        int off[4];
#pragma unroll
        for (int u = 0; u < 4; ++u) off[u] = kb0 + 64 * u < NK ? trow[kb0 + 64 * u] : -1;
        if (nsplit == 1) {
#pragma unroll
            for (int hh = 0; hh < 4; ++hh) {
                if (hh >= hg) break;
                float v[4];
#pragma unroll
                for (int u = 0; u < 4; ++u) v[u] = off[u] >= 0 ? dh[hh * hstride + off[u]] : 0.f;
                a[hh] += (v[0] + v[1]) + (v[2] + v[3]);
            }
        } else {
#pragma unroll
            for (int u = 0; u < 4; ++u) {
                if (off[u] < 0) continue;
                const float* pe = dh + off[u];
                int sp = 0;
                for (; sp + 4 <= nsplit; sp += 4)
                    a[0] += (pe[sp * split_stride] + pe[(sp + 1) * split_stride]) +
                            (pe[(sp + 2) * split_stride] + pe[(sp + 3) * split_stride]);
                for (; sp < nsplit; ++sp) a[0] += pe[sp * split_stride];
            }
        }
    }
#pragma unroll
    for (int hh = 0; hh < 4; ++hh) {
        if (hh >= hg) break;
        const float t = wave_sum(a[hh]);
        if (lane == 0) static_cast<float*>(en.dtable)[slot * en.nH + h0 + hh] += t;
    }
}

constexpr int F32_MAXT = 16;
__global__ void __launch_bounds__(256) attn_f32_fwd_kernel(const float* __restrict__ q, const float* __restrict__ k,
                                                           const float* __restrict__ v, float* __restrict__ o,
                                                           const float* __restrict__ table, const int* __restrict__ rid,
                                                           const float* __restrict__ kmask, Geom G, int round_p) {
    extern __shared__ __attribute__((aligned(16))) unsigned char smem[];
    const int N = G.g.N, hd = G.g.hd;
    int* row_s = reinterpret_cast<int*>(smem);
    int* lin_s = row_s + N;
    int* rid_s = lin_s + N;
    float* kadd_s = reinterpret_cast<float*>(rid_s + N);
    float* p_s = kadd_s + N;
    const int tid = threadIdx.x, lane = tid & 63, wave = tid >> 6;
    const int gh = blockIdx.x, grp = gh / G.g.nH, h = gh - grp * G.g.nH;
    const int wloc = (G.g.mode == 1) ? grp % G.nW : 0;
    for (int n = tid; n < N; n += 256) {
        row_s[n] = (int)tok_row(G, grp, n);
        lin_s[n] = (G.g.mode == 1 && table) ? win_lin(G, n) : 0;
        rid_s[n] = (G.g.mode == 1 && rid) ? rid[wloc * N + n] : 0;
        kadd_s[n] = (G.g.mode == 0 && kmask) ? kmask[(int64_t)grp * N + n] : 0.f;
    }
    __syncthreads();
    float* pw = p_s + wave * N;
    for (int qi = blockIdx.y * 4 + wave; qi < N; qi += 4 * gridDim.y) {
        const float* qp = q + (int64_t)row_s[qi] * G.g.ldq + h * hd;
        const int linq = lin_s[qi] + G.tcst + G.tb0, rq = rid_s[qi];
        float s[F32_MAXT];
        float m = -INFINITY;
#pragma unroll
        for (int t = 0; t < F32_MAXT; ++t) {
            const int j = t * 64 + lane;
            s[t] = -INFINITY;
            if (j < N) {
                const float* kp = k + (int64_t)row_s[j] * G.g.ldk + h * hd;
                float dot = 0.f;
                for (int d = 0; d < hd; d += 4) {
                    const float4 a = *reinterpret_cast<const float4*>(qp + d);
                    const float4 b = *reinterpret_cast<const float4*>(kp + d);
                    dot = fmaf(a.x, b.x, dot); dot = fmaf(a.y, b.y, dot);
                    dot = fmaf(a.z, b.z, dot); dot = fmaf(a.w, b.w, dot);
                }
                float sc = dot * G.g.scale;
                if (G.g.mode == 1 && table) sc += table[(int64_t)(linq - lin_s[j]) * G.g.nH + h];
                if (G.g.mode == 1 && rid && rid_s[j] != rq) sc += -100.0f;
                sc += kadd_s[j];
                s[t] = sc;
                m = fmaxf(m, sc);
            }
        }
        m = wave_max(m);
        float sum = 0.f;
#pragma unroll
        for (int t = 0; t < F32_MAXT; ++t) {
            const int j = t * 64 + lane;
            if (j < N) {
                float e = expf(s[t] - m);
                if (round_p == 1) e = bf2f(f2bf(e));
                else if (round_p == 2) e = (float)(_Float16)e;
                s[t] = e;
                sum += e;
            }
        }
        sum = wave_sum(sum);
        const float inv = 1.0f / sum;
#pragma unroll
        for (int t = 0; t < F32_MAXT; ++t) {
            const int j = t * 64 + lane;
            if (j < N) pw[j] = s[t];
        }
        __builtin_amdgcn_wave_barrier();
        if (lane < hd) {
            float acc = 0.f;
            for (int j = 0; j < N; ++j) acc = fmaf(pw[j], v[(int64_t)row_s[j] * G.g.ldv + h * hd + lane], acc);
            o[(int64_t)row_s[qi] * G.g.ldo + h * hd + lane] = acc * inv;
        }
        __builtin_amdgcn_wave_barrier();
    }
}

template <bool PASS_K>
__global__ void __launch_bounds__(256) attn_f32_bwd_kernel(const float* __restrict__ q, const float* __restrict__ k,
// ... 207 lines not shown
        if (g->mode == 0 && tiles > SEQ_ONE_PART_TILES && g->N <= SEQ_MAX_KEYS) {
            G.nparts = (tiles + SEQ_ONE_PART_TILES - 1) / SEQ_ONE_PART_TILES;
            G.pt16 = (tiles + G.nparts - 1) / G.nparts * 16;
            G.tsplit = G.nparts;
            static_assert(SEQ_MAX_PARTS * SEQ_ONE_PART_TILES * 16 >= SEQ_MAX_KEYS, "parts cover the longest sequence");
            if ((G.nparts - 1) * G.pt16 >= g->N) return false;
            const int64_t tokens = (int64_t)g->groups * g->N, C = (int64_t)g->nH * g->hd;
            G.o_ps = tokens * C;
            G.lse_ps = (int64_t)g->groups * g->nH * g->N;
            G.lddq = G.lddk = G.lddv = (int)C;
            G.dq_ps = G.dk_ps = G.dv_ps = 3 * tokens * C;
        }
    }
    if (g->mode == 1) {
        if (g->wd <= 0 || g->wh <= 0 || g->ww <= 0) return false;
        if (g->D % g->wd || g->H % g->wh || g->W % g->ww) return false;
        if (g->N != g->wd * g->wh * g->ww) return false;
        G.nWh = g->H / g->wh;
        G.nWw = g->W / g->ww;
        G.nW = (g->D / g->wd) * G.nWh * G.nWw;
        if (g->groups % G.nW) return false;
        if (g->sd < 0 || g->sd >= g->D || g->sh < 0 || g->sh >= g->H || g->sw < 0 || g->sw >= g->W) return false;
        if (g->bwd || g->bwh || g->bww) {
            if (g->bwd <= 0 || g->bwh <= 0 || g->bww <= 0) return false;
            G.ts_h = 2 * g->bww - 1;
            G.ts_d = (2 * g->bwh - 1) * G.ts_h;
            G.tlen = (2 * g->bwd - 1) * G.ts_d;
            G.tb0 = g->wd < g->bwd ? (g->bwd - g->wd) * G.ts_d : 0;
            G.tbn = g->wd < g->bwd ? (2 * g->wd - 1) * G.ts_d : G.tlen;
            G.tcst = (g->bwd - 1) * G.ts_d + (g->bwh - 1) * G.ts_h + (g->bww - 1) - G.tb0;
            G.tls = (G.tbn + 3) / 4 * 4;
            if (g->N > g->bwd * g->bwh * g->bww) return false;
        }
    } else if (g->mode != 0) {
        return false;
    }
    return true;
}

constexpr size_t MAX_LDS = 160 * 1024;
constexpr int DBIAS_SPLITS = 32;

inline int dbias_splits(const Geom& G) {
    int splits = G.g.groups / DBIAS_GROUPS_PER_SLICE;
    return splits < 1 ? 1 : (splits > DBIAS_SPLITS ? DBIAS_SPLITS : splits);
}
inline int64_t ds_scratch_bytes(const Geom& G, int nkt) {
    const int64_t b = (int64_t)G.g.groups * G.g.nH * ((G.g.N + 15) / 16) * nkt * 256 * 2;
    return (b + 255) / 256 * 256;
}

template <int HD, int NKT>
size_t fwd_lds(int tls, bool window = false) { return 2 * (size_t)(NKT * 16) * (HD + 8) * 2 + (window ? 3 : 4) * (size_t)NKT * 16 * 4 + (size_t)tls * 4 + 16; }
template <int HD, int NKT>
size_t dq_lds(int tls) { return 2 * (size_t)(NKT * 16) * (HD + 8) * 2 + 4 * (size_t)NKT * 16 * 4 + (size_t)tls * 4 + 16; }
template <int HD, int NKT>
size_t dkv_lds(int tls) { return 2 * (size_t)(NKT * 16) * (HD + 8) * 2 + 5 * (size_t)NKT * 16 * 4 + (size_t)tls * 4 + 16; }

#define CLV_PICK_N(KERNEL, NT, ...)                                                                    \
    do {                                                                                               \
        if (G.g.mode == 1) { KERNEL<HD, NT, false, 1> __VA_ARGS__; }                                   \
        else if (G.drop_thresh) { KERNEL<HD, NT, true, 0> __VA_ARGS__; }                               \
        else { KERNEL<HD, NT, false, 0> __VA_ARGS__; }                                                 \
    } while (0)
#define CLV_PICK(KERNEL, ...) CLV_PICK_N(KERNEL, NKT, __VA_ARGS__)

template <int HD, int NKT>
void set_attrs() {
    static bool done = false;
    if (done) return;
    done = true;
#define CLV_ATTR(K) (void)hipFuncSetAttribute(reinterpret_cast<const void*>(&K), hipFuncAttributeMaxDynamicSharedMemorySize, (int)MAX_LDS)
    CLV_ATTR((attn_fwd_kernel<HD, NKT, false, 1>));
    CLV_ATTR((attn_fwd_kernel<HD, NKT, false, 0>));
    CLV_ATTR((attn_fwd_kernel<HD, NKT, true, 0>));
    CLV_ATTR((attn_bwd_dq_kernel<HD, NKT, false, 1>));
    CLV_ATTR((attn_bwd_dq_kernel<HD, NKT, false, 0>));
    CLV_ATTR((attn_bwd_dq_kernel<HD, NKT, true, 0>));
    constexpr int NKE = (NKT + 1) & ~1;
    CLV_ATTR((attn_bwd_dkv_kernel<HD, NKE, false, 1>));
    CLV_ATTR((attn_bwd_dkv_kernel<HD, NKE, false, 0>));
    CLV_ATTR((attn_bwd_dkv_kernel<HD, NKE, true, 0>));
    if constexpr (HD == 32 && (NKT == 13 || NKT == 25)) CLV_ATTR((attn_bwd_one_kernel<HD, NKT>));
#undef CLV_ATTR
}

template <int HD, int NKT>
int launch_fwd(const void* q, const void* k, const void* v, void* o, float* lse, const float* bias,
               const int32_t* rid, const float* kmask, const unsigned long long* seed, const Geom& G, hipStream_t st) {
    const int bl = bias ? G.tls : 0;
    const size_t lds = fwd_lds<HD, NKT>(bl, G.g.mode == 1);
    if (lds > MAX_LDS || dq_lds<HD, NKT>(bl) > MAX_LDS || dkv_lds<HD, NKT>(bl) > MAX_LDS) return CLV_ERR_UNSUPPORTED;
    if (G.g.mode == 1 && G.drop_thresh) return CLV_ERR_UNSUPPORTED;
    set_attrs<HD, NKT>();
    const int nblk = G.g.groups * G.g.nH * G.tsplit * G.nparts;
    if (G.nparts == 1) {
        CLV_PICK(attn_fwd_kernel, <<<dim3(nblk), dim3(THREADS), lds, st>>>((const bf16_t*)q, (const bf16_t*)k,
                 (const bf16_t*)v, (bf16_t*)o, lse, bias, rid, kmask, seed, G));
        return clv_check_launch();
    }
    if (!G.g.work || (NKT + WAVES - 1) / WAVES * WAVES * G.tsplit < (G.g.N + 15) / 16) return CLV_ERR_UNSUPPORTED;
    Geom P = G;
    P.g.ldo = G.g.nH * G.g.hd;
    bf16_t* o_part = reinterpret_cast<bf16_t*>(G.g.work);
    float* lse_part = reinterpret_cast<float*>(o_part + G.nparts * G.o_ps);
    CLV_PICK(attn_fwd_kernel, <<<dim3(nblk), dim3(THREADS), lds, st>>>((const bf16_t*)q, (const bf16_t*)k,
             (const bf16_t*)v, o_part, lse_part, bias, rid, kmask, seed, P));
    int rc = clv_check_launch();
    if (rc) return rc;
    const int64_t items = (int64_t)G.g.groups * G.g.N * (G.g.nH * G.g.hd / 8);
    hipLaunchKernelGGL(seq_combine_fwd_kernel, dim3((unsigned)((items + 255) / 256)), dim3(256), 0, st, o_part, lse_part,
                       (bf16_t*)o, lse, G);
    return clv_check_launch();
}

template <int HD, int NKT>
bool one_eligible(const Geom& G, bool has_bias) {
    if constexpr (HD == 32 && (NKT == 13 || NKT == 25)) {
        const int one_mode = clv_env_int("CLV_ATTN_BWD_ONE", 1);
        return one_mode > 0 && G.g.mode == 1 && G.nparts == 1 && !G.drop_thresh &&
               (G.tsplit == 1 || G.g.groups * G.g.nH >= 192 || one_mode > 1) && (G.g.N + 15) / 16 == NKT && has_bias &&
               G.tbn <= 3 * (ONE_CWAVES(NKT) + ONE_SWAVES(NKT)) * 64 && one_lds<HD, NKT>(G.tls) <= MAX_LDS;
    }
    return false;
}
template <int HD, int NKT>
int query_one(const Geom& G) { return one_eligible<HD, NKT>(G, true) ? 1 : 0; }

template <int HD, int NKT>
int launch_bwd(const void* q, const void* k, const void* v, const void* o, const void* dout,
               const float* lse, const float* bias, const int32_t* rid, const float* kmask, void* dq,
               void* dk, void* dv, float* dbias, float* dsum, void* work, const unsigned long long* seed, int stages,
               const Geom& G, hipStream_t st) {
    const int bl = bias ? G.tls : 0;
    constexpr int NKE = (NKT + 1) & ~1;
    const size_t lds_a = dq_lds<HD, NKT>(bl), lds_b = dkv_lds<HD, NKE>(bl);
    if (lds_a > MAX_LDS || lds_b > MAX_LDS) return CLV_ERR_UNSUPPORTED;
    if (G.g.mode == 1 && G.drop_thresh) return CLV_ERR_UNSUPPORTED;
    set_attrs<HD, NKT>();
    const int nblk = G.g.groups * G.g.nH * G.tsplit * G.nparts;
    int rc = CLV_OK;
    bf16_t* dq_out = (bf16_t*)dq;
    bf16_t* dk_out = (bf16_t*)dk;
    bf16_t* dv_out = (bf16_t*)dv;
    if (G.nparts > 1) {
        const int looped = (G.g.N + 15) / 16;
        if (!G.g.work || (NKT + DKV_THREADS(NKT) / 64 - 1) / (DKV_THREADS(NKT) / 64) * (DKV_THREADS(NKT) / 64) * G.tsplit < looped ||
            (NKE + DKV_THREADS(NKE) / 64 - 1) / (DKV_THREADS(NKE) / 64) * (DKV_THREADS(NKE) / 64) * G.tsplit < looped)
            return CLV_ERR_UNSUPPORTED;
        const int64_t tc = (int64_t)G.g.groups * G.g.N * G.g.nH * G.g.hd;
        dq_out = reinterpret_cast<bf16_t*>(G.g.work);
        dk_out = dq_out + tc;
        dv_out = dq_out + 2 * tc;
    }
    const bool one = one_eligible<HD, NKT>(G, bias != nullptr) && (stages & 5) == 5;
    auto launch_one = [&](const Geom& Gx, int groups) {
        if constexpr (HD == 32 && (NKT == 13 || NKT == 25))
            attn_bwd_one_kernel<HD, NKT><<<dim3(groups * G.g.nH), dim3((ONE_CWAVES(NKT) + ONE_SWAVES(NKT)) * 64), one_lds<HD, NKT>(bl), st>>>(
                (const bf16_t*)q, (const bf16_t*)k, (const bf16_t*)v, (const bf16_t*)o, (const bf16_t*)dout, lse, bias, rid,
                dq_out, dk_out, dv_out, (bf16_t*)(bias ? work : nullptr), dsum, Gx);
    };
    const int64_t E = (int64_t)G.g.nH * ((G.g.N + 15) / 16) * NKT * 64;
    float* partial = !bias ? nullptr
                     : G.g.work ? reinterpret_cast<float*>(G.g.work)
                                : reinterpret_cast<float*>(reinterpret_cast<char*>(work) + ds_scratch_bytes(G, NKT));
    const int splits = dbias_splits(G);
    int nch = 1;
    if (bias && (stages & 7) == 7 && G.nparts == 1) {
        const int64_t per_group = E * 2;
        while (nch < 8 && (G.g.groups / nch) * per_group > (int64_t)DBIAS_CHUNK_MB << 20 && G.g.groups % (2 * nch) == 0 &&
               splits % (2 * nch) == 0)
            nch *= 2;
    }
    if (nch > 1) {
        const int cg = G.g.groups / nch, spc = splits / nch;
        for (int cix = 0; cix < nch; ++cix) {
            Geom Cg = G;
            Cg.grp0 = cix * cg;
            const int nb = cg * G.g.nH * G.tsplit;
            if (one) launch_one(Cg, cg);
            else
            CLV_PICK(attn_bwd_dq_kernel, <<<dim3(nb), dim3(DKV_THREADS(NKT)), lds_a, st>>>((const bf16_t*)q, (const bf16_t*)k,
                     (const bf16_t*)v, (const bf16_t*)o, (const bf16_t*)dout, lse, bias, rid, kmask, dq_out,
                     (bf16_t*)work, dsum, seed, Cg));
            hipLaunchKernelGGL(dbias_sum_kernel, dim3((unsigned)((E / 2 + 255) / 256), spc), dim3(256), 0, st,
                               (const bf16_t*)work, reinterpret_cast<float4*>(partial + (int64_t)cix * spc * E * 4), cg, E / 2);
        }
        rc = clv_check_launch();
        if (rc) return rc;
    } else if (one) {
        launch_one(G, G.g.groups);
        rc = clv_check_launch();
        if (rc) return rc;
    } else if (stages & 1) {
        CLV_PICK(attn_bwd_dq_kernel, <<<dim3(nblk), dim3(DKV_THREADS(NKT)), lds_a, st>>>((const bf16_t*)q, (const bf16_t*)k,
                 (const bf16_t*)v, (const bf16_t*)o, (const bf16_t*)dout, lse, bias, rid, kmask, dq_out,
                 (bf16_t*)(bias ? work : nullptr), dsum, seed, G));
        rc = clv_check_launch();
        if (rc) return rc;
    }
    if (bias && (stages & 2)) {
        float* dense = partial + (int64_t)splits * E * 4;
        if (nch == 1)
            hipLaunchKernelGGL(dbias_sum_kernel, dim3((unsigned)((E / 2 + 255) / 256), splits), dim3(256), 0, st,
                               (const bf16_t*)work, reinterpret_cast<float4*>(partial), G.g.groups, E / 2);
        (void)dense;
        if (stages & 8) {
        } else if (G.g.dbias_index) {
            hipLaunchKernelGGL(dbias_gather_tab_kernel, dim3((G.tbn * G.g.nH + 3) / 4), dim3(256), 0, st, partial, dbias,
                               G.g.dbias_index, NKT, G, splits, E * 4, G.tb0, G.tbn);
        }
        else
            hipLaunchKernelGGL(dbias_gather_kernel, dim3((G.tlen * G.g.nH + 3) / 4), dim3(256), 0, st, partial, dbias, NKT, G,
                               splits, E * 4);
        rc = clv_check_launch();
        if (rc) return rc;
    }
    if ((stages & 4) && !one) {
        CLV_PICK_N(attn_bwd_dkv_kernel, NKE, <<<dim3(nblk), dim3(DKV_THREADS(NKE)), lds_b, st>>>((const bf16_t*)q, (const bf16_t*)k,
                 (const bf16_t*)v, (const bf16_t*)dout, lse, dsum, bias, rid, kmask, dk_out, dv_out, seed, G));
        rc = clv_check_launch();
        if (rc) return rc;
        if (G.nparts > 1) {
            const int64_t items = 3 * (int64_t)G.g.groups * G.g.N * (G.g.nH * G.g.hd / 8);
            hipLaunchKernelGGL(seq_combine_bwd_kernel, dim3((unsigned)((items + 255) / 256)), dim3(256), 0, st,
                               reinterpret_cast<const bf16_t*>(G.g.work), (bf16_t*)dq, (bf16_t*)dk, (bf16_t*)dv, G);
            rc = clv_check_launch();
        }
    }
    return rc;
}

int pick_nkt(int N) {
    const int need = (N + 15) / 16;
    const int opts[] = {2, 8, 13, 14, 15, 16, 25, 28};
    for (int o : opts) if (o >= need) return o;
    return -1;
}

#define DISPATCH_NKT(HDV, FN, ...)                                   \
    switch (nkt) {                                                   \
        case 2: return FN<HDV, 2>(__VA_ARGS__);                      \
        case 8: return FN<HDV, 8>(__VA_ARGS__);                      \
        case 13: return FN<HDV, 13>(__VA_ARGS__);                    \
        case 14: return FN<HDV, 14>(__VA_ARGS__);                    \
        case 15: return FN<HDV, 15>(__VA_ARGS__);                    \
        case 16: return FN<HDV, 16>(__VA_ARGS__);                    \
        case 25: return FN<HDV, 25>(__VA_ARGS__);                    \
        case 28: return FN<HDV, 28>(__VA_ARGS__);                    \
        default: return CLV_ERR_UNSUPPORTED;                         \
    }

}

extern "C" int clv_attn_fwd(const void* q, const void* k, const void* v, void* o, float* lse,
                            const float* bias, const int32_t* rid, const float* kmask, const void* seed,
                            const ClvAttnGeom* geom, void* stream) {
    Geom G;
    if (!q || !k || !v || !o || !lse || !make_geom(geom, G)) return CLV_ERR_ARG;
    if (G.drop_thresh && !seed) return CLV_ERR_ARG;
    const unsigned long long* sp = (const unsigned long long*)seed;
    if (bias && (G.g.mode != 1 || G.tlen == 0)) return CLV_ERR_ARG;
    if (rid && G.g.mode != 1) return CLV_ERR_ARG;
    const int nkt = pick_nkt(G.nparts > 1 ? G.pt16 : G.g.N);
    hipStream_t st = (hipStream_t)stream;
    if (G.g.hd == 16) { DISPATCH_NKT(16, launch_fwd, q, k, v, o, lse, bias, rid, kmask, sp, G, st) }
    if (G.g.hd == 32) { DISPATCH_NKT(32, launch_fwd, q, k, v, o, lse, bias, rid, kmask, sp, G, st) }
    DISPATCH_NKT(64, launch_fwd, q, k, v, o, lse, bias, rid, kmask, sp, G, st)
}

extern "C" int64_t clv_attn_bwd_work_bytes(const ClvAttnGeom* geom) {
    Geom G;
    if (!make_geom(geom, G) || G.g.mode != 1 || G.tlen == 0) return 0;
    const int nkt = pick_nkt(G.g.N);
    if (nkt < 0) return 0;
    return ds_scratch_bytes(G, nkt) + (int64_t)(DBIAS_SPLITS + 1) * G.g.nH * ((G.g.N + 15) / 16) * nkt * 256 * 4;
}

extern "C" int64_t clv_attn_dbias_partial_bytes(const ClvAttnGeom* geom) {
    Geom G;
    if (!make_geom(geom, G) || G.g.mode != 1 || G.tlen == 0) return 0;
    const int nkt = pick_nkt(G.g.N);
    if (nkt < 0) return 0;
    return (int64_t)dbias_splits(G) * G.g.nH * ((G.g.N + 15) / 16) * nkt * 256 * 4;
}

extern "C" int clv_attn_bwd_one_kernel(const ClvAttnGeom* geom) {
    Geom G;
    if (!make_geom(geom, G) || G.g.mode != 1 || G.tlen == 0 || G.g.hd != 32) return 0;
    const int nkt = pick_nkt(G.g.N);
    DISPATCH_NKT(32, query_one, G)
}

extern "C" int64_t clv_attn_seq_work_bytes(const ClvAttnGeom* geom) {
    Geom G;
    if (!make_geom(geom, G) || G.nparts == 1) return 0;
    const int64_t tc = (int64_t)G.g.groups * G.g.N * G.g.nH * G.g.hd;
    const int64_t fwd = G.nparts * (tc * 2 + G.lse_ps * 4), bwd = G.nparts * 3 * tc * 2;
    return fwd > bwd ? fwd : bwd;
}

extern "C" int clv_attn_seq_max_keys(void) { return SEQ_MAX_KEYS; }

extern "C" int clv_attn_seq_parts(const ClvAttnGeom* geom) {
    Geom G;
    if (!make_geom(geom, G) || pick_nkt(G.nparts > 1 ? G.pt16 : G.g.N) < 0) return 0;
    return G.nparts;
}

extern "C" int64_t clv_attn_dbias_index_count(const ClvAttnGeom* geom) {
    Geom G;
    if (!make_geom(geom, G) || G.g.mode != 1 || G.tlen == 0) return 0;
    return (int64_t)G.tlen * pick_nkt(G.g.N) * 16;
}

extern "C" int clv_attn_dbias_index(const ClvAttnGeom* geom, int32_t* out, void* stream) {
    Geom G;
    if (!out || !make_geom(geom, G) || G.g.mode != 1 || G.tlen == 0) return CLV_ERR_ARG;
    const int nkt = pick_nkt(G.g.N);
    const int64_t n = (int64_t)G.tlen * nkt * 16;
    hipLaunchKernelGGL(dbias_index_kernel, dim3((unsigned)((n + 255) / 256)), dim3(256), 0, (hipStream_t)stream, out, nkt, G);
    return clv_check_launch();
}

extern "C" int clv_attn_bwd(const void* q, const void* k, const void* v, const void* o, const void* dout,
                            const float* lse, const float* bias, const int32_t* rid, const float* kmask,
                            void* dq, void* dk, void* dv, float* dbias, float* dsum, void* work,
                            const void* seed, int32_t stages, const ClvAttnGeom* geom, void* stream) {
    Geom G;
    const unsigned long long* sp = (const unsigned long long*)seed;
    if (stages == 0) stages = 7;
    if (!q || !k || !v || !o || !dout || !lse || !dq || !dk || !dv || !dsum || !make_geom(geom, G)) return CLV_ERR_ARG;
    if (bias && (G.g.mode != 1 || G.tlen == 0 || !dbias || !work)) return CLV_ERR_ARG;
    if (rid && G.g.mode != 1) return CLV_ERR_ARG;
    if (G.drop_thresh && !seed) return CLV_ERR_ARG;
    const int nkt = pick_nkt(G.nparts > 1 ? G.pt16 : G.g.N);
    hipStream_t st = (hipStream_t)stream;
    if (G.g.hd == 16) { DISPATCH_NKT(16, launch_bwd, q, k, v, o, dout, lse, bias, rid, kmask, dq, dk, dv, dbias, dsum, work, sp, stages, G, st) }
    if (G.g.hd == 32) { DISPATCH_NKT(32, launch_bwd, q, k, v, o, dout, lse, bias, rid, kmask, dq, dk, dv, dbias, dsum, work, sp, stages, G, st) }
    DISPATCH_NKT(64, launch_bwd, q, k, v, o, dout, lse, bias, rid, kmask, dq, dk, dv, dbias, dsum, work, sp, stages, G, st)
}


extern "C" int clv_attn_dbias_gather_entry(const ClvAttnGeom* geom, void* work, float* dbias, ClvDbiasGather* out) {
    Geom G;
    if (!geom || !work || !dbias || !out || !make_geom(geom, G) || G.g.mode != 1 || G.tlen == 0 || !G.g.dbias_index)
        return CLV_ERR_ARG;
    const int nkt = pick_nkt(G.g.N);
    if (nkt < 0) return CLV_ERR_UNSUPPORTED;
    const int64_t E = (int64_t)G.g.nH * ((G.g.N + 15) / 16) * nkt * 64;
    out->partial = G.g.work ? reinterpret_cast<char*>(G.g.work) : reinterpret_cast<char*>(work) + ds_scratch_bytes(G, nkt);
    out->dtable = dbias;
    out->index = G.g.dbias_index;
    out->split_stride = E * 4;
    out->nkt = nkt;
    out->nH = G.g.nH;
    out->N = G.g.N;
    out->nsplit = dbias_splits(G);
    out->slot0 = G.tb0;
    out->nslots = G.tbn;
    out->block_begin = 0;
    out->pad = 0;
    return CLV_OK;
}

extern "C" int clv_attn_dbias_gather_batch(const ClvDbiasGather* entries, int32_t n, void* stream) {
    if (!entries || n <= 0 || n > CLV_DBIAS_GATHER_MAX) return CLV_ERR_ARG;
    static_assert(sizeof(ClvDbiasGather) == 64, "ClvDbiasGather layout is part of the ABI");
    GatherTable tab;
    int blocks = 0;
    for (int i = 0; i < n; ++i) {
        ClvDbiasGather en = entries[i];
        if (!en.partial || !en.dtable || !en.index || en.nsplit <= 0 || en.nslots <= 0 || en.nH <= 0) return CLV_ERR_ARG;
        tab.e[i] = en;
    }
    tab.n = n;
    for (int i = 0; i < n; ++i) {
        ClvDbiasGather& en = tab.e[i];
        int hg = 1;
        for (int c = DBIAS_HEADS_PER_WAVE; c >= 2; --c)
            if (en.nH % c == 0) { hg = c; break; }
        en.pad = hg;
        en.block_begin = blocks;
        blocks += (en.nslots * (en.nH / hg) + 3) / 4;
    }
    GatherTable st = tab;
    int sblocks = 0;
    bool any = false;
    for (int i = 0; i < n; ++i) {
        if ((st.e[i].split_stride & 3) || (reinterpret_cast<uintptr_t>(st.e[i].partial) & 15)) return CLV_ERR_ARG;
        st.e[i].block_begin = sblocks;
        sblocks += (int)(((st.e[i].split_stride >> 2) + 255) / 256);
        any |= st.e[i].nsplit > 1;
        tab.e[i].nsplit = 1;
    }
    if (any) {
        hipLaunchKernelGGL(dbias_split_sum_batch_kernel, dim3((unsigned)sblocks), dim3(256), 0, (hipStream_t)stream, st);
        const int rc = clv_check_launch();
        if (rc) return rc;
    }
    hipLaunchKernelGGL(dbias_gather_batch_kernel, dim3((unsigned)blocks), dim3(256), 0, (hipStream_t)stream, tab);
    return clv_check_launch();
}

extern "C" int clv_attn_f32_fwd(const float* q, const float* k, const float* v, float* o, const float* bias,
                                const int32_t* rid, const float* kmask, const ClvAttnGeom* geom, int32_t round_p,
                                void* stream) {
    Geom G;
    if (!q || !k || !v || !o || !make_geom(geom, G)) return CLV_ERR_ARG;
    if (bias && (G.g.mode != 1 || G.tlen == 0)) return CLV_ERR_ARG;
    if (rid && G.g.mode != 1) return CLV_ERR_ARG;
    if (G.g.N > F32_MAXT * 64 || G.drop_thresh) return CLV_ERR_UNSUPPORTED;
    const size_t lds = (size_t)G.g.N * (4 * 4 + 4 * 4);
    const int pairs = G.g.groups * G.g.nH;
    int ysplit = 1;
    while (pairs * ysplit < 2048 && ysplit * 8 <= G.g.N) ysplit *= 2;
    hipLaunchKernelGGL(attn_f32_fwd_kernel, dim3(pairs, ysplit), dim3(256), lds, (hipStream_t)stream, q, k, v, o, bias, rid,
                       kmask, G, round_p);
    return clv_check_launch();
}

extern "C" int64_t clv_attn_f32_bwd_work_floats(const ClvAttnGeom* geom) {
    Geom G;
// ... 28 lines not shown
```

### clover_amd/ops.py

```python
import ctypes as C

import os
from typing import Any, NamedTuple, Optional

import torch

from . import _lib, parity
from ._lib import ClvAttnGeom, check

BF16 = _lib.half_dtype()


def _stream():
    return C.c_void_p(torch.cuda.current_stream().cuda_stream)


def _ptr(t):
    return C.c_void_p(t.data_ptr()) if t is not None else C.c_void_p(0)


def _need_gpu(*ts):
    for t in ts:
        if t is not None and not t.is_cuda:
            raise RuntimeError('clover_amd ops run only on a HIP device (MI355X); there is no CPU fallback — '
# ... 1317 lines not shown
            raise ValueError('Expected more than 1 value per channel when training')
        y = torch.empty_like(x2)
        mean = torch.empty(D, device=x2.device, dtype=torch.float32)
        rstd = torch.empty_like(mean)
        check(_lib.lib().clv_batchnorm1d_fwd(_ptr(x2), _ptr(weight), _ptr(bias), _ptr(running_mean), _ptr(running_var),
                                             _ptr(y), _ptr(mean), _ptr(rstd), B, D, float(eps), float(momentum),
                                             int(bool(training)), _stream()), 'clv_batchnorm1d_fwd')
        ctx.save_for_backward(x2, weight, mean, rstd)
        ctx.training = bool(training)
        ctx.has_bias = bias is not None
        return y

    @staticmethod
    def backward(ctx, dy):
        x2, weight, mean, rstd = ctx.saved_tensors
        B, D = x2.shape
        dy2 = _c(dy.float())
        dx = torch.empty_like(x2) if ctx.needs_input_grad[0] else None
        dg = torch.empty(D, device=x2.device, dtype=torch.float32) if weight is not None else None
        db = torch.empty(D, device=x2.device, dtype=torch.float32) if ctx.has_bias else None
        check(_lib.lib().clv_batchnorm1d_bwd(_ptr(dy2), _ptr(x2), _ptr(weight), _ptr(mean), _ptr(rstd), _ptr(dx), _ptr(dg),
                                             _ptr(db), B, D, int(ctx.training), _stream()), 'clv_batchnorm1d_bwd')
        return dx, dg, db, None, None, None, None, None


def batch_norm1d(x, weight, bias, running_mean, running_var, training, momentum=0.1, eps=1e-5):
    return _BatchNorm1d.apply(x, weight, bias, running_mean, running_var, training, momentum, eps)


class _TokenMean(torch.autograd.Function):

    @staticmethod
    def forward(ctx, x):
        ctx.shape, ctx.dtype = x.shape, x.dtype
        return x.mean(dim=tuple(range(1, x.dim() - 1)), dtype=torch.float32)

    @staticmethod
    def backward(ctx, g):
        shape = ctx.shape
        n = 1
        for d in shape[1:-1]:
            n *= d
        gs = (g * (1.0 / n)).to(ctx.dtype)
        return gs.view((shape[0],) + (1,) * (len(shape) - 2) + (shape[-1],)).expand(shape)


def token_mean(x):
    if x.dim() < 3:
        return x.float()
    return _TokenMean.apply(x)


class _Embedding(torch.autograd.Function):

    @staticmethod
    def forward(ctx, ids, weight, padding_idx):
        ctx.save_for_backward(ids)
        ctx.wref, ctx.pad = weight, padding_idx
        return weight.detach()[ids]

    @staticmethod
    def backward(ctx, dy):
        (ids,) = ctx.saved_tensors
        w = ctx.wref
        sink = _sink(w)
        flat = ids.reshape(-1)
        d = dy.reshape(-1, dy.shape[-1])
        if ctx.pad is not None:
            d = d.masked_fill((flat == ctx.pad)[:, None], 0)
        if sink is not None:
            sink.index_add_(0, flat, d.float())
            _delivered(w)
            return None, None, None
        return None, torch.zeros_like(w).index_add_(0, flat, d.to(w.dtype)), None


def embedding(ids, weight, padding_idx=None):
    return _Embedding.apply(ids, weight, padding_idx)


class _Attention(torch.autograd.Function):

    @staticmethod
    def forward(ctx, qkv, table, rid, kmask, geom_kw, seed):
        _need_gpu(qkv)
        assert qkv.dtype == BF16 and qkv.is_contiguous()
        g = ClvAttnGeom(**geom_kw)
        assert g.dropout_p == 0.0 or seed is not None
        Cdim = g.nH * g.hd
        assert qkv.shape[-1] == 3 * Cdim
        g.ldq = g.ldk = g.ldv = 3 * Cdim
        g.ldo = Cdim
        tab = None
        if table is not None:
            assert table.shape == ((2 * g.bwd - 1) * (2 * g.bwh - 1) * (2 * g.bww - 1), g.nH), table.shape
            tab = _c(table.detach().float())
        o = torch.empty(qkv.shape[:-1] + (Cdim,), device=qkv.device, dtype=BF16)
        lse = torch.empty(g.groups * g.nH * g.N, device=qkv.device, dtype=torch.float32)
        wbytes = _lib.lib().clv_attn_seq_work_bytes(C.byref(g))
        seq_work = torch.empty(wbytes, device=qkv.device, dtype=torch.uint8) if wbytes > 0 else None
        g.work = seq_work.data_ptr() if seq_work is not None else None
        base = qkv.data_ptr()
        with _Timed(_kname('attn_fwd_kernel', g), *_attn_work(g, False)):
            check(_lib.lib().clv_attn_fwd(C.c_void_p(base), C.c_void_p(base + 2 * Cdim),
                                          C.c_void_p(base + 4 * Cdim), _ptr(o), _ptr(lse), _ptr(tab), _ptr(rid),
                                          _ptr(kmask), _ptr(seed), C.byref(g), _stream()), 'clv_attn_fwd')
        ctx.save_for_backward(qkv, o, lse, tab, rid, kmask, seed)
        ctx.geom = g
        ctx.tref = table
        return o

    @staticmethod
    def backward(ctx, do):
        qkv, o, lse, tab, rid, kmask, seed = ctx.saved_tensors
        g = ctx.geom
        Cdim = g.nH * g.hd
        doc = _c(do)
        if doc.dtype != BF16:
            doc = doc.to(BF16)
        dqkv = torch.empty_like(qkv)
        dsum = torch.empty_like(lse)
        L = _lib.lib()
        wbytes = L.clv_attn_seq_work_bytes(C.byref(g))
        seq_work = torch.empty(wbytes, device=qkv.device, dtype=torch.uint8) if wbytes > 0 else None
        g.work = seq_work.data_ptr() if seq_work is not None else None
        dtab = work = sink = None
        if tab is not None:
            sink = _sink(ctx.tref)
            dtab = sink if sink is not None else torch.zeros_like(tab)
            work = torch.empty(L.clv_attn_bwd_work_bytes(C.byref(g)), device=qkv.device, dtype=torch.uint8)
            g.dbias_index = _dbias_index(g, qkv.device)
        b, d = qkv.data_ptr(), dqkv.data_ptr()
        args = (C.c_void_p(b), C.c_void_p(b + 2 * Cdim), C.c_void_p(b + 4 * Cdim), _ptr(o), _ptr(doc), _ptr(lse),
                _ptr(tab), _ptr(rid), _ptr(kmask), C.c_void_p(d), C.c_void_p(d + 2 * Cdim),
                C.c_void_p(d + 4 * Cdim), _ptr(dtab), _ptr(dsum), _ptr(work), _ptr(seed))
        if PROF is None and SEGMENT is not None and sink is not None:
            part = torch.empty(L.clv_attn_dbias_partial_bytes(C.byref(g)), device=qkv.device, dtype=torch.uint8)
            g.work = part.data_ptr()
            check(L.clv_attn_bwd(*args, 15, C.byref(g), _stream()), 'clv_attn_bwd')
            ent = _lib.ClvDbiasGather()
            check(L.clv_attn_dbias_gather_entry(C.byref(g), _ptr(work), _ptr(dtab), C.byref(ent)), 'clv_attn_dbias_gather_entry')
            g.work = None
            SEGMENT.dbias.append(DbiasItem(ent, part, dtab, g.dbias_index))
        elif PROF is None:
            check(L.clv_attn_bwd(*args, 0, C.byref(g), _stream()), 'clv_attn_bwd')
        elif tab is not None and L.clv_attn_bwd_one_kernel(C.byref(g)) == 1:
            fl, by = _attn_work(g, True)
            with _Timed(f'attn_bwd_one_kernel<{g.hd}, {(g.N + 15) // 16}>', fl, by):
                check(L.clv_attn_bwd(*args, 5, C.byref(g), _stream()), 'clv_attn_bwd')
            check(L.clv_attn_bwd(*args, 2, C.byref(g), _stream()), 'clv_attn_bwd')
        else:
            fl, by = _attn_work(g, True)
            with _Timed(_kname('attn_bwd_dq_kernel', g), fl * 0.4, by * 0.5):
                check(L.clv_attn_bwd(*args, 1, C.byref(g), _stream()), 'clv_attn_bwd')
            check(L.clv_attn_bwd(*args, 2, C.byref(g), _stream()), 'clv_attn_bwd')
            with _Timed(_kname('attn_bwd_dkv_kernel', g), fl * 0.6, by * 0.5):
                check(L.clv_attn_bwd(*args, 4, C.byref(g), _stream()), 'clv_attn_bwd')
        if sink is not None:
            _delivered(ctx.tref)
            dtab = None
        elif dtab is not None:
            dtab = dtab.to(ctx.tref.dtype)
        return dqkv, dtab, None, None, None, None


def window_attention(qkv, table, rid, window, shift, num_heads, table_window=None):
    B, D, H, W, C3 = qkv.shape
    Cdim = C3 // 3
    hd = Cdim // num_heads
    N = window[0] * window[1] * window[2]
    nW = (D // window[0]) * (H // window[1]) * (W // window[2])
    tw = tuple(table_window or window) if table is not None else (0, 0, 0)
    kw = dict(mode=1, groups=B * nW, N=N, nH=num_heads, hd=hd, D=D, H=H, W=W, wd=window[0], wh=window[1],
              ww=window[2], sd=shift[0], sh=shift[1], sw=shift[2], bwd=tw[0], bwh=tw[1], bww=tw[2],
              scale=float(hd) ** -0.5)
    if parity.enabled():
        return parity.attention(qkv, table, rid, None, kw)
    return _Attention.apply(qkv, table, rid, None, kw, None)


_DROPOUT_COUNTER = {}


_SEED_STRIDE = 0x9E3779B97F4A7C15 - (1 << 64)
_SEED_POOL = {}


def _dev_key(device):
    d = torch.device(device)
    return f'cuda:{torch.cuda.current_device() if d.index is None else d.index}' if d.type == 'cuda' else str(d)


def _wrap64(v):
    v &= (1 << 64) - 1
    return v - (1 << 64) if v >= (1 << 63) else v


def dropout_seeds_begin(device, n=128):
    key = _dev_key(device)
    ctr = _dropout_counter(device)
    pool = _SEED_POOL.get(key)
    if pool is None or pool['seeds'].numel() != n:
        pool = dict(seeds=torch.empty(n, device=device, dtype=torch.int64),
                    steps=torch.arange(n, device=device, dtype=torch.int64) * _SEED_STRIDE, idx=0)
        _SEED_POOL[key] = pool
    torch.add(pool['steps'], ctr, out=pool['seeds'])
    ctr.add_(_wrap64(n * _SEED_STRIDE))
    pool['idx'] = 0


def dropout_seeds_end(device):
    _SEED_POOL.pop(_dev_key(device), None)


def _dropout_counter(device):
    key = _dev_key(device)
    if key not in _DROPOUT_COUNTER:
        init = int(torch.randint(1, 2 ** 62, (1,)).item())
        _DROPOUT_COUNTER[key] = torch.tensor([init], device=device, dtype=torch.int64)
    return _DROPOUT_COUNTER[key]


def next_dropout_seed(device):
    pool = _SEED_POOL.get(_dev_key(device))
    if pool is not None and pool['idx'] < pool['seeds'].numel():
        i = pool['idx']
        pool['idx'] = i + 1
        return pool['seeds'][i:i + 1]
    ctr = _dropout_counter(device)
    seed = ctr.clone()
    ctr.add_(_SEED_STRIDE)
    return seed


SEQ_FUSED_MAX_KEYS = _lib.lib().clv_attn_seq_max_keys()


class _LongSeqAttention(torch.autograd.Function):

    @staticmethod
    def forward(ctx, qkv, kmask, num_heads, dropout_p, seed):
        _need_gpu(qkv)
        assert qkv.dtype == BF16
        B, S, C3 = qkv.shape
        Cdim = C3 // 3
        hd = Cdim // num_heads
        q, k, v = (qkv[..., i * Cdim:(i + 1) * Cdim].view(B, S, num_heads, hd).permute(0, 2, 1, 3) for i in range(3))
        _library_gemm('seq_attention (more than %d keys)' % SEQ_FUSED_MAX_KEYS, (B, num_heads, S, hd))
        scores = torch.matmul(q, k.transpose(-1, -2))
        p = torch.empty_like(scores)
        pd = torch.empty_like(scores) if dropout_p > 0 else None
        km = _c(kmask.float()) if kmask is not None else None
        scale = float(hd) ** -0.5
        check(_lib.lib().clv_softmax_rows_fwd(_ptr(scores), _ptr(km), _ptr(p), _ptr(pd), _ptr(seed),
                                              B * num_heads * S, S, S, num_heads * S, scale, float(dropout_p),
                                              _stream()), 'clv_softmax_rows_fwd')
        o = torch.matmul(pd if pd is not None else p, v)
        ctx.save_for_backward(qkv, p, pd, seed)
        ctx.cfg = (num_heads, hd, scale, float(dropout_p))
        return o.permute(0, 2, 1, 3).reshape(B, S, Cdim)

    @staticmethod
    def backward(ctx, do):
        qkv, p, pd, seed = ctx.saved_tensors
        num_heads, hd, scale, dropout_p = ctx.cfg
        B, S, C3 = qkv.shape
        Cdim = C3 // 3
        q, k, v = (qkv[..., i * Cdim:(i + 1) * Cdim].view(B, S, num_heads, hd).permute(0, 2, 1, 3) for i in range(3))
        doh = do.to(BF16).view(B, S, num_heads, hd).permute(0, 2, 1, 3)
        dqkv = torch.empty_like(qkv)
        dq, dk, dv = (dqkv[..., i * Cdim:(i + 1) * Cdim].view(B, S, num_heads, hd).permute(0, 2, 1, 3) for i in range(3))
        dv.copy_(torch.matmul((pd if pd is not None else p).transpose(-1, -2), doh))
        ds = torch.matmul(doh, v.transpose(-1, -2))
        check(_lib.lib().clv_softmax_rows_bwd(_ptr(p), _ptr(ds), _ptr(ds), _ptr(seed), B * num_heads * S, S, S,
                                              scale, dropout_p, _stream()), 'clv_softmax_rows_bwd')
        dq.copy_(torch.matmul(ds, k))
        dk.copy_(torch.matmul(ds.transpose(-1, -2), q))
        return dqkv, None, None, None, None


def seq_attention(qkv, kmask, num_heads, dropout_p=0.0):
    B, S, C3 = qkv.shape
    hd = C3 // 3 // num_heads
    if parity.enabled():
        return parity.attention(qkv, None, None, kmask, dict(mode=0, groups=B, N=S, nH=num_heads, hd=hd,
                                                            scale=float(hd) ** -0.5, dropout_p=float(dropout_p)))
    if S > SEQ_FUSED_MAX_KEYS:
        seed = next_dropout_seed(qkv.device) if dropout_p > 0 else None
        return _LongSeqAttention.apply(qkv, kmask, num_heads, float(dropout_p), seed)
    kw = dict(mode=0, groups=B, N=S, nH=num_heads, hd=hd, scale=float(hd) ** -0.5, dropout_p=float(dropout_p))
    seed = next_dropout_seed(qkv.device) if dropout_p > 0 else None
    return _Attention.apply(qkv, None, None, kmask, kw, seed)


class _PatchEmbed(torch.autograd.Function):
    @staticmethod
    def forward(ctx, x, weight, bias, gamma, beta, mask_token, vmask, want_clean, eps, stacked=False):
        _need_gpu(x, weight)
        B, Cin, T, H, W = x.shape
        Cout = weight.shape[0]
        assert Cin == 3 and tuple(weight.shape[1:]) == (3, 2, 4, 4), 'kernel covers patch (2,4,4), 3 input channels'
        xc = _c(x.float())
        w2 = _c(weight.reshape(Cout, 96).to(BF16))
        bf = _c(bias.float())
        gf = _c(gamma.float()) if gamma is not None else None
        bef = _c(beta.float()) if beta is not None else None
        want_masked = vmask is not None
        mt = _c(mask_token.reshape(-1).float()) if want_masked else None
        vm = _c(vmask.reshape(B, vmask.shape[-2], vmask.shape[-1]).long()) if want_masked else None
        Tp, Hp, Wp = T // 2, H // 4, W // 4
        M = B * Tp * Hp * Wp
        dev = x.device
        need_grad = any(t is not None and t.requires_grad for t in (weight, bias, gamma, beta, mask_token))
        both = None
        if stacked:
            assert want_clean and want_masked
            both = torch.empty(2 * B, Tp, Hp, Wp, Cout, device=dev, dtype=BF16)
            clean, masked = both[:B], both[B:]
        else:
            clean = torch.empty(B, Tp, Hp, Wp, Cout, device=dev, dtype=BF16) if want_clean else None
            masked = torch.empty(B, Tp, Hp, Wp, Cout, device=dev, dtype=BF16) if want_masked else None
        z = torch.empty(M, Cout, device=dev, dtype=BF16) if need_grad else None
        mean = torch.empty(M, device=dev, dtype=torch.float32) if need_grad else None
        rstd = torch.empty(M, device=dev, dtype=torch.float32) if need_grad else None
        mh, mw = (vm.shape[1], vm.shape[2]) if want_masked else (1, 1)
        if FP8:
            w8, wsc = quant_fp8_rows(w2)
            check(_lib.lib().clv_patch_embed_fwd_fp8(_ptr(xc), _ptr(w8), _ptr(wsc), _ptr(bf), _ptr(gf), _ptr(bef), _ptr(mt),
                                                     _ptr(vm), _ptr(clean), _ptr(masked), _ptr(z), _ptr(mean), _ptr(rstd),
                                                     B, T, H, W, Cout, mh, mw, float(eps), _stream()),
                  'clv_patch_embed_fwd_fp8')
        else:
            check(_lib.lib().clv_patch_embed_fwd(_ptr(xc), _ptr(w2), _ptr(bf), _ptr(gf), _ptr(bef), _ptr(mt), _ptr(vm),
                                                 _ptr(clean), _ptr(masked), _ptr(z), _ptr(mean), _ptr(rstd), B, T, H, W,
                                                 Cout, mh, mw, float(eps), _stream()), 'clv_patch_embed_fwd')
        ctx.save_for_backward(xc, z, mean, rstd, gf, vm)
        ctx.prefs = (weight, bias, gamma, beta, mask_token)
        ctx.meta = (B, T, H, W, Cout, want_clean, want_masked, weight.shape,
                    mask_token.shape if mask_token is not None else None)
        ctx.stacked = bool(stacked)
        if stacked:
            return both, x.new_empty(0)
        outs = (clean if want_clean else x.new_empty(0), masked if want_masked else x.new_empty(0))
        return outs

    @staticmethod
    def backward(ctx, dclean, dmasked):
        xc, z, mean, rstd, gf, vm = ctx.saved_tensors
        B, T, H, W, Cout, want_clean, want_masked, wshape, mtshape = ctx.meta
        Tp, Hp, Wp = T // 2, H // 4, W // 4
        M = B * Tp * Hp * Wp
        L = _lib.lib()

        def bf(t):
            return _half_rows(t, Cout) if t is not None else None
        if ctx.stacked:
            dclean, dmasked = (dclean[:B], dclean[B:]) if dclean is not None else (None, None)
        dc = bf(dclean) if want_clean else None
        dm = bf(dmasked) if want_masked else None
        dmt = None
        weight, bias, gamma, beta, mask_token = ctx.prefs
        ps = (weight, bias, gamma, beta, mask_token if dm is not None else None)
        sinks = _sinks(*ps)
        sink = sinks is not None
        if sink:
            wsink, bsink, gsink, besink, msink = sinks
        if dm is None:
            dyb = dc
        else:
            dyb = torch.empty(M, Cout, device=xc.device, dtype=BF16)
            dmt = msink.view(-1) if sink else torch.zeros(Cout, device=xc.device, dtype=torch.float32)
            check(L.clv_patch_embed_blend_bwd(_ptr(dc), _ptr(dm), _ptr(vm), _ptr(dyb), _ptr(dmt), B, T, H, W, Cout,
                                              vm.shape[1], vm.shape[2], _stream()), 'clv_patch_embed_blend_bwd')
            dmt = None if sink else dmt.reshape(mtshape)
        if gf is not None:
# ... 772 lines not shown
```

### include/clover_hip.h

```cpp
#ifndef CLOVER_HIP_H
#define CLOVER_HIP_H
#include <stdint.h>

#ifdef __cplusplus
extern "C" {
#endif

#define CLV_ABI_VERSION 18
#define CLV_ERR_ARG (-1)
#define CLV_ERR_UNSUPPORTED (-2)
#define CLV_ERR_LAUNCH (-3)

int clv_abi_version(void);
int clv_half_type(void);

typedef struct ClvAttnGeom {
    int32_t mode;
    int32_t groups;
    int32_t N;
    int32_t nH;
    int32_t hd;
    int32_t D, H, W;
    int32_t wd, wh, ww;
    int32_t sd, sh, sw;
    int32_t ldq, ldk, ldv, ldo;
    int32_t bwd, bwh, bww;
    float scale;
    float dropout_p;
    const int32_t* dbias_index;
    void* work;
} ClvAttnGeom;

int64_t clv_attn_seq_work_bytes(const ClvAttnGeom* geom);
int clv_attn_seq_max_keys(void);
int clv_attn_seq_parts(const ClvAttnGeom* geom);
int clv_attn_fwd(const void* q, const void* k, const void* v, void* o, float* lse,
                 const float* bias, const int32_t* rid, const float* kmask, const void* seed,
                 const ClvAttnGeom* geom_host, void* stream);

int64_t clv_attn_bwd_work_bytes(const ClvAttnGeom* geom_host);
int clv_attn_bwd_one_kernel(const ClvAttnGeom* geom_host);
int64_t clv_attn_dbias_index_count(const ClvAttnGeom* geom_host);
int clv_attn_dbias_index(const ClvAttnGeom* geom_host, int32_t* out, void* stream);
int clv_attn_bwd(const void* q, const void* k, const void* v, const void* o, const void* dout,
                 const float* lse, const float* bias, const int32_t* rid, const float* kmask,
                 void* dq, void* dk, void* dv, float* dbias, float* dsum, void* work,
                 const void* seed, int32_t stages, const ClvAttnGeom* geom_host, void* stream);
#define CLV_DBIAS_GATHER_MAX 32
typedef struct ClvDbiasGather {
    const void* partial;
    void* dtable;
    const void* index;
    int64_t split_stride;
    int32_t nkt, nH, N, nsplit, slot0, nslots, block_begin, pad;
} ClvDbiasGather;
int clv_attn_dbias_gather_entry(const ClvAttnGeom* geom_host, void* work, float* dbias, ClvDbiasGather* out);
int64_t clv_attn_dbias_partial_bytes(const ClvAttnGeom* geom_host);
int clv_attn_dbias_gather_batch(const ClvDbiasGather* entries, int32_t n, void* stream);

int clv_softmax_rows_fwd(const void* scores, const float* kmask, void* p, void* pd, const void* seed, int64_t rows,
                         int32_t S, int32_t ld, int32_t rows_per_group, float scale, float dropout_p, void* stream);
int clv_softmax_rows_bwd(const void* p, const void* dpd, void* ds, const void* seed, int64_t rows, int32_t S,
                         int32_t ld, float scale, float dropout_p, void* stream);

typedef struct ClvLnExtra {
    const float* xscale;
    int32_t rows_per_sample;
    float drop_p;
    const void* seed;
    const void* dy2;
    void* dres;
    int32_t x_is_sum;
    int32_t gather_c, gather_h2, gather_w2;
    int32_t no_reduce;
    void* q8;
    float* qscale;
} ClvLnExtra;
int clv_layernorm_fwd(const void* x, const void* res, const float* gamma, const float* beta,
                      void* y, void* sum_out, float* mean, float* rstd, int64_t rows, int32_t C,
                      float eps, int32_t is_f32, const ClvLnExtra* extra, void* stream);
int clv_layernorm_bwd_blocks(int64_t rows, int32_t C);
int clv_layernorm_bwd(const void* dy, const void* x, const void* res, const float* gamma,
                      const float* mean, const float* rstd, const void* dsum, void* dx, float* dgamma, float* dbeta,
                      float* partial, int64_t rows, int32_t C, int32_t is_f32, const ClvLnExtra* extra, void* stream);

#define CLV_LN_REDUCE_MAX 64
typedef struct ClvLnReduceEntry {
    const float* partial;
    float* dgamma;
    float* dbeta;
    int32_t nblk, C, block_begin, pad;
} ClvLnReduceEntry;
int clv_layernorm_bwd_needs_reduce(int64_t rows, int32_t C);
int clv_ln_reduce_batch(const ClvLnReduceEntry* entries, int32_t n, void* stream);

int clv_ln_fold_fwd(const float* w, const float* b, const float* gamma, const float* beta, void* wf, float* bf,
                    int32_t N, int32_t K, void* stream);
int clv_ln_fold_bwd(const float* dwf, const float* dbf, const float* w, const float* gamma, const float* beta,
                    float* dw, float* db, float* dgamma, float* dbeta, int32_t N, int32_t K, void* stream);

int clv_batchnorm1d_fwd(const float* x, const float* gamma, const float* beta, float* running_mean, float* running_var,
                        float* y, float* save_mean, float* save_rstd, int32_t B, int32_t D, float eps, float momentum,
                        int32_t training, void* stream);
int clv_batchnorm1d_bwd(const float* dy, const float* x, const float* gamma, const float* save_mean, const float* save_rstd,
                        float* dx, float* dgamma, float* dbeta, int32_t B, int32_t D, int32_t training, void* stream);

int clv_gelu_fwd(const void* x, void* y, int64_t n, int32_t is_f32, void* stream);
int clv_gelu_bwd(const void* dy, const void* x, void* dx, int64_t n, int32_t is_f32, void* stream);

int clv_patch_embed_fwd(const float* x, const void* w, const float* bias, const float* gamma,
                        const float* beta, const float* mask_token, const int64_t* vmask,
                        void* out_clean, void* out_masked, void* z_out, float* mean, float* rstd,
                        int32_t B, int32_t T, int32_t H, int32_t W, int32_t C, int32_t mh,
                        int32_t mw, float eps, void* stream);
int clv_patch_embed_blend_bwd(const void* dclean, const void* dmasked, const int64_t* vmask, void* dy,
                              float* dmask_token, int32_t B, int32_t T, int32_t H, int32_t W, int32_t C,
                              int32_t mh, int32_t mw, void* stream);
int clv_im2col_patches(const float* x, void* patches, int32_t B, int32_t T, int32_t H, int32_t W,
                       void* stream);

int64_t clv_linear_wgrad_work_floats(int64_t M, int32_t N, int32_t K);
int clv_linear_wgrad(const void* dy, const void* x, float* dw, float* db, float* work, int64_t M,
                     int32_t N, int32_t K, int32_t ldy, int32_t ldx, const float* xmean,
                     const float* xrstd, int32_t stages, void* stream);
#define CLV_FOLD_MAX 64
typedef struct ClvFoldEntry {
    const void* partial;
    void* dw;
    void* db;
    int64_t nk, e2;
    int32_t splits, sg_shift, block_begin;
    int32_t overwrite;
} ClvFoldEntry;
typedef struct ClvWgradEntry {
    const void* dy;
    const void* x;
    void* work;
    float* dw;
    float* db;
    int64_t M, work_floats;
    int32_t N, K, ldy, ldx, want_bias, splits;
// ... 209 lines not shown
```

Baseline: 758.5 pairs/s.

## Precompute per-pattern bias+mask images for Swin window attention kernels

```diff
diff --git a/clover_amd/_lib.py b/clover_amd/_lib.py
--- a/clover_amd/_lib.py
+++ b/clover_amd/_lib.py
@@ -54,6 +54,14 @@
 
 
 DBIAS_GATHER_MAX = 32
+
+
+class ClvAttnImgEntry(C.Structure):
+    _fields_ = [('geom', C.POINTER(ClvAttnGeom)), ('table', _p), ('rid', _p), ('pmap', _p), ('img', _p),
+                ('npat', _i32), ('fwd_only', _i32)]
+
+
+ATTN_IMG_MAX = 16
 
 
 class ClvLnReduceEntry(C.Structure):
@@ -85,6 +93,12 @@
     'clv_attn_dbias_partial_bytes': (C.c_int64, [_p]),
     'clv_attn_dbias_gather_batch': (C.c_int, [C.POINTER(ClvDbiasGather), _i32, _p]),
     'clv_attn_bwd': (C.c_int, [_p] * 16 + [_i32, C.POINTER(ClvAttnGeom), _p]),
+    'clv_attn_img_supported': (C.c_int, [C.POINTER(ClvAttnGeom)]),
+    'clv_attn_img_wins': (C.c_int, [C.POINTER(ClvAttnGeom)]),
+    'clv_attn_img_floats': (C.c_int64, [C.POINTER(ClvAttnGeom), _i32]),
+    'clv_attn_img_build_batch': (C.c_int, [C.POINTER(ClvAttnImgEntry), _i32, _p]),
+    'clv_attn_fwd_img': (C.c_int, [_p] * 9 + [C.POINTER(ClvAttnGeom), _p]),
+    'clv_attn_bwd_img': (C.c_int, [_p] * 16 + [_i32, C.POINTER(ClvAttnGeom), _p]),
     'clv_softmax_rows_fwd': (C.c_int, [_p] * 5 + [_i64, _i32, _i32, _i32, _f, _f, _p]),
     'clv_softmax_rows_bwd': (C.c_int, [_p] * 4 + [_i64, _i32, _i32, _f, _f, _p]),
     'clv_layernorm_fwd': (C.c_int, [_p] * 8 + [_i64, _i32, _f, _i32, C.POINTER(ClvLnExtra), _p]),
diff --git a/clover_amd/backbones/swin_transformer_3d.py b/clover_amd/backbones/swin_transformer_3d.py
--- a/clover_amd/backbones/swin_transformer_3d.py
+++ b/clover_amd/backbones/swin_transformer_3d.py
@@ -1,3 +1,5 @@
+import ctypes as C
+import weakref
 from functools import lru_cache
 
 import numpy as np
@@ -6,7 +8,7 @@
 import torch.nn.functional as F
 import torch.utils.checkpoint as _checkpoint
 
-from .. import ops
+from .. import _lib, ops
 from ..builder import BACKBONES
 from ..nn import GELU, DropPath, LayerNorm, Linear, trunc_normal_
 
@@ -65,6 +67,31 @@
 def window_geometry(x_size, cfg_ws, cfg_ss, device):
     ws, ss, rid, _ = _window_geometry_cached(tuple(x_size), tuple(cfg_ws), tuple(cfg_ss), str(device))
     return ws, ss, rid
+
+
+def window_pattern_map(rid):
+    rid = np.asarray(rid)
+    pmap = np.zeros(rid.shape[0], dtype=np.int32)
+    seen = {}
+    for w, row in enumerate(rid):
+        _, first, inv = np.unique(row, return_index=True, return_inverse=True)
+        canon = np.argsort(np.argsort(first))[inv.reshape(-1)]
+        if canon.max() > 0:
+            pmap[w] = seen.setdefault(canon.astype(np.int32).tobytes(), len(seen) + 1)
+    return pmap, len(seen) + 1
+
+
+@lru_cache(maxsize=64)
+def _window_patterns_cached(x_size, cfg_ws, cfg_ss, device_str):
+    ws, ss, rid, _ = _window_geometry_cached(x_size, cfg_ws, cfg_ss, device_str)
+    if rid is None:
+        return None, 1
+    pmap, npat = window_pattern_map(rid.cpu().numpy())
+    return torch.from_numpy(pmap).to(device_str), npat
+
+
+def window_patterns(x_size, cfg_ws, cfg_ss, device):
+    return _window_patterns_cached(tuple(x_size), tuple(cfg_ws), tuple(cfg_ss), str(device))
 
 
 def gathered_bias(table, rel_index, N):
@@ -121,12 +148,13 @@
             lin.weight._clv_want_t = ops.wants_transposed(lin.out_features, lin.in_features)
         self.proj_drop = nn.Dropout(proj_drop)
         trunc_normal_(self.relative_position_bias_table, std=.02)
+        self.image = None
 
     def forward(self, x, ws, ss, rid):
         N = ws[0] * ws[1] * ws[2]
         qkv = self.qkv(x)
         o = ops.window_attention(qkv, self.relative_position_bias_table, rid if any(s > 0 for s in ss) else None,
-                                 ws, ss, self.num_heads, table_window=self.window_size)
+                                 ws, ss, self.num_heads, table_window=self.window_size, image=self.image)
         return self.proj_drop(self.proj(o))
 
 
@@ -201,7 +229,7 @@
             qkv, s0 = ops.ln_linear(branch, x, self.norm1.weight, self.norm1.bias, at.qkv.weight, at.qkv.bias,
                                     self.norm1.eps)
         o = ops.window_attention(qkv, at.relative_position_bias_table, rid if any(s > 0 for s in ss) else None, ws, ss,
-                                 self.num_heads, table_window=at.window_size)
+                                 self.num_heads, table_window=at.window_size, image=at.image)
         a = at.proj(o)
         m, s1 = ops.fused_mlp(a, s0, self.norm2.weight, self.norm2.bias, self.mlp.fc1.weight, self.mlp.fc1.bias,
                               self.mlp.fc2.weight, self.mlp.fc2.bias, self.norm2.eps, x_scale=self._dp_scale(a))
@@ -316,6 +344,9 @@
     def forward(self, x):
         clean, _ = self.tokens(x)
         return clean.permute(0, 4, 1, 2, 3)
+
+
+_IMG_PLANS = weakref.WeakKeyDictionary()
 
 
 @BACKBONES.register_module()
@@ -444,8 +475,78 @@
         mods = list(self.layers[self.CUT_STAGE:]) + [self.norm]
         return [q for m in mods for q in m.parameters()]
 
+    def _attn_image_plan(self, x):
+        key = (str(x.device),) + tuple(x.shape)
+        plans = _IMG_PLANS.setdefault(self, {})
+        plan = plans.get(key)
+        if plan is not None or torch.cuda.is_current_stream_capturing():
+            return plan
+        L = _lib.lib()
+        B, D, H, W, Cdim = x.shape
+        items, total = [], 0
+        for layer in self.layers:
+            for blk in layer.blocks:
+                ws, ss, rid = window_geometry((D, H, W), blk.window_size, blk.shift_size, x.device)
+                pd, ph, pw = (-(-n // w) * w for n, w in zip((D, H, W), ws))
+                kw = ops.window_attention_kw(B, pd, ph, pw, Cdim, ws, ss, blk.num_heads, blk.attn.window_size)
+                g = _lib.ClvAttnGeom(**kw)
+                g.ldq = g.ldk = g.ldv = 3 * Cdim
+                g.ldo = Cdim
+                shifted = any(s > 0 for s in ss)
+                pmap, npat = window_patterns((D, H, W), blk.window_size, blk.shift_size, x.device) if shifted else (None, 1)
+                n = L.clv_attn_img_floats(C.byref(g), npat) if L.clv_attn_img_wins(C.byref(g)) == 1 else 0
+                if n > 0:
+                    items.append((blk.attn, g, rid if shifted else None, pmap, npat, total, n, ops.attn_image_key(kw)))
+                    total += n
+            if layer.downsample is not None:
+                H, W, Cdim = (H + 1) // 2, (W + 1) // 2, 2 * Cdim
+        buf = torch.empty(total, device=x.device, dtype=torch.float32)
+        plan = plans[key] = dict(buf=buf, items=items, tables=None, calls=[], images=[
+            (it[0], ops.AttnImage(buf[it[5]:it[5] + it[6]], it[3], it[7], backward=False)) for it in items])
+        return plan
+
+    def _build_attn_images(self, x):
+        if not x.is_cuda or ops.parity.enabled():
+            return None
+        plan = self._attn_image_plan(x)
+        if plan is None or not plan['items']:
+            return None
+        tabs = [it[0].relative_position_bias_table for it in plan['items']]
+        if any(t.dtype != torch.float32 or not t.is_contiguous() or t.device != x.device for t in tabs):
+            return None
+        ptrs = tuple(t.data_ptr() for t in tabs)
+        if plan['tables'] != ptrs:
+            plan['calls'] = []
+            for c0 in range(0, len(tabs), _lib.ATTN_IMG_MAX):
+                chunk = plan['items'][c0:c0 + _lib.ATTN_IMG_MAX]
+                arr = (_lib.ClvAttnImgEntry * len(chunk))()
+                for e, it, p in zip(arr, chunk, ptrs[c0:]):
+                    e.geom = C.pointer(it[1])
+                    e.table = p
+                    e.rid = it[2].data_ptr() if it[2] is not None else None
+                    e.pmap = it[3].data_ptr() if it[3] is not None else None
+                    e.img = plan['buf'].data_ptr() + 4 * it[5]
+                    e.npat = it[4]
+                    e.fwd_only = 1
+                plan['calls'].append(arr)
+            plan['tables'] = ptrs
+        st = C.c_void_p(torch.cuda.current_stream().cuda_stream)
+        for arr in plan['calls']:
+            _lib.check(_lib.lib().clv_attn_img_build_batch(arr, len(arr), st), 'clv_attn_img_build_batch')
+        return plan['images']
+
     def _stages(self, x, mid_cut=None):
         self._draw_drop_paths(x.shape[0], x.device)
+        images = self._build_attn_images(x)
+        for attn, image in images or ():
+            attn.image = image
+        try:
+            return self._stages_body(x, mid_cut)
+        finally:
+            for attn, _ in images or ():
+                attn.image = None
+
+    def _stages_body(self, x, mid_cut=None):
         x = self.pos_drop(x)
         for i, layer in enumerate(self.layers[:-1]):
             if mid_cut is not None and i == self.CUT_STAGE:
diff --git a/clover_amd/csrc/attention.hip b/clover_amd/csrc/attention.hip
--- a/clover_amd/csrc/attention.hip
+++ b/clover_amd/csrc/attention.hip
@@ -129,8 +129,11 @@
 constexpr float LOG2E = 1.4426950408889634f;
 __device__ __forceinline__ float exp_sub(float x, float negL2) { return __builtin_amdgcn_exp2f(fmaf(x, LOG2E, negL2)); }
 
-template <int HD, int NKT, bool DROP, int MODE>
-__global__ void __launch_bounds__(THREADS, (NKT <= 16 ? 3 : 1)) attn_fwd_kernel(
+constexpr bool IMG_SHAPE(int hd, int nkt) { return hd == 32 && nkt == 13; }
+constexpr int IMG_TILES(int nkt) { return nkt * nkt + ((nkt + 1) & ~1) * nkt; }
+
+template <int HD, int NKT, bool DROP, int MODE, bool IMG = false>
+__global__ void __launch_bounds__(THREADS, (NKT <= 16 ? (IMG ? 4 : 3) : 1)) attn_fwd_kernel(
     const bf16_t* __restrict__ q, const bf16_t* __restrict__ k, const bf16_t* __restrict__ v,
     bf16_t* __restrict__ o, float* __restrict__ lse, const float* __restrict__ bias,
     const int* __restrict__ rid, const float* __restrict__ kmask, const unsigned long long* __restrict__ seedp,
@@ -153,7 +156,8 @@
     int* linb_s = row_s + NK;
     float* tab_s = reinterpret_cast<float*>(linb_s + NK);
     int* flag_s = reinterpret_cast<int*>(tab_s + G.tls);
-    if (tid == 0) *flag_s = 0;
+    static_assert(!IMG || (MODE == 1 && NKT <= 16 && !DROP), "image variant: window mode, one softmax chunk");
+    if (!IMG && tid == 0) *flag_s = 0;
     token_rows<NK>(G, grp, row_s, tid, THREADS, s0);
     constexpr int PRE = NKT <= 16 ? (NKT + WAVES - 1) / WAVES : 1;
     const int nqt = (N + 15) >> 4;
@@ -167,14 +171,25 @@
             load_frags<HD>(qpre[ti], q + loop_row(G, row_s, grp, qv ? nq : 0) * G.g.ldq + h * HD, qv, lane);
         }
     }
+    const int wloc = (G.g.mode == 1) ? grp % G.nW : 0;
+    const float4* imq = nullptr;
+    float4 im[IMG ? NKT : 1];
+    if (IMG) {
+        const int pc = rid ? rid[wloc] : 0;
+        imq = reinterpret_cast<const float4*>(bias) + (int64_t)(pc * G.g.nH + h) * (IMG_TILES(NKT) * 64) + lane;
+        const int qt0 = wave + WAVES * part;
+        if (qt0 < nqt) {
+#pragma unroll
+            for (int t = 0; t < (IMG ? NKT : 1); ++t) im[t] = imq[(qt0 * NKT + t) * 64];
+        }
+    }
     stage<HD, NK, true>(row_s, k, G.g.ldk, h, Ns, Ks, tid, THREADS, G.g.scale * LOG2E);
     stage<HD, NK>(row_s, v, G.g.ldv, h, Ns, Vs, tid);
-    if (MODE == 1 && bias) load_bias_table<NK>(G, bias, h, tab_s, linb_s, tid, THREADS, LOG2E);
+    if (!IMG && MODE == 1 && bias) load_bias_table<NK>(G, bias, h, tab_s, linb_s, tid, THREADS, LOG2E);
     int* rid_s = reinterpret_cast<int*>(aux);
     float* kadd = aux + NK;
-    const int wloc = (G.g.mode == 1) ? grp % G.nW : 0;
     int differs = 0;
-    for (int n = tid; n < NK; n += THREADS) {
+    for (int n = tid; n < (IMG ? 0 : NK); n += THREADS) {
         if (MODE == 1 && rid) {
             const int rv = (n < N) ? rid[wloc * N + n] : 0;
             rid_s[n] = rv;
@@ -182,9 +197,9 @@
         }
         if (MODE == 0) kadd[n] = (n < Ns) ? (kmask ? kmask[(int64_t)grp * N + s0 + n] * LOG2E : 0.f) : -INFINITY;
     }
-    if (differs) *flag_s = 1;
+    if (!IMG && differs) *flag_s = 1;
     __syncthreads();
-    const bool masked = *flag_s != 0;
+    const bool masked = IMG ? false : *flag_s != 0;
 
     const int lg = lane >> 4, lr = lane & 15;
     Frag8 onesf;
@@ -207,9 +222,9 @@
 
         constexpr int CH = NKT > 16 ? 14 : NKT;
         float p[CH][4];
-        const bool tb = MODE == 1 && bias != nullptr;
+        const bool tb = !IMG && MODE == 1 && bias != nullptr;
         const char* tp = reinterpret_cast<const char*>(tab_s) + (tb ? linb_s[qv ? nq : 0] + 4 * G.tcst : 0);
-        const int rq = (MODE == 1 && rid && qv) ? rid_s[nq] : 0;
+        const int rq = (!IMG && MODE == 1 && rid && qv) ? rid_s[nq] : 0;
         float4 bnext = make_float4(0.f, 0.f, 0.f, 0.f);
         if (tb) bnext = table_bias4(tp, linb_s + lg * 4);
         f32x4_t oacc[NC];
@@ -229,14 +244,14 @@
                 Frag8 kf[KS];
                 lds_frags<HD>(kf, Ks + (t * 16 + lr) * LDR, lane);
                 const int key0 = t * 16 + lg * 4;
-                asm volatile("" ::: "memory");
-                const float4 bv = bnext;
+                if (!IMG) asm volatile("" ::: "memory");
+                const float4 bv = IMG ? im[IMG ? t : 0] : bnext;
                 if (tb && t + 1 < NKT) bnext = table_bias4(tp, linb_s + (t + 1) * 16 + lg * 4);
                 f32x4_t acc = {bv.x, bv.y, bv.z, bv.w};
                 if (MODE == 0) {
                     const float4 ka = *reinterpret_cast<const float4*>(kadd + key0);
                     acc[0] += ka.x; acc[1] += ka.y; acc[2] += ka.z; acc[3] += ka.w;
-                } else if ((t + 1) * 16 > Ns) {
+                } else if (!IMG && (t + 1) * 16 > Ns) {
 #pragma unroll
                     for (int r = 0; r < 4; ++r) acc[r] = (key0 + r < Ns) ? acc[r] : -INFINITY;
                 }
@@ -304,6 +319,11 @@
                 pf.u[1] = pack2bf(p[2 * s2][2], p[2 * s2][3]);
                 pf.u[2] = tail ? 0u : pack2bf(p[tail ? 0 : 2 * s2 + 1][0], p[tail ? 0 : 2 * s2 + 1][1]);
                 pf.u[3] = tail ? 0u : pack2bf(p[tail ? 0 : 2 * s2 + 1][2], p[tail ? 0 : 2 * s2 + 1][3]);
+                if (IMG && ti + 1 < (NKT + WAVES - 1) / WAVES) {
+                    const float4* imn = imq + min(qt + WAVES * G.tsplit, nqt - 1) * (NKT * 64);
+                    im[IMG ? 2 * s2 : 0] = imn[(2 * s2) * 64];
+                    if (!tail) im[IMG && !tail ? 2 * s2 + 1 : 0] = imn[(2 * s2 + 1) * 64];
+                }
                 const int kt = c0 + 2 * s2;
 #pragma unroll
                 for (int c = 0; c < NC; ++c) {
@@ -691,7 +711,7 @@
 
 __device__ __forceinline__ void lds_barrier() { asm volatile("s_waitcnt lgkmcnt(0)\n\ts_barrier" ::: "memory"); }
 
-template <int HD, int NKT>
+template <int HD, int NKT, bool IMG = false>
 __global__ void __launch_bounds__((ONE_CWAVES(NKT) + ONE_SWAVES(NKT)) * 64, ONE_MINW) attn_bwd_one_kernel(
     const bf16_t* __restrict__ q, const bf16_t* __restrict__ k, const bf16_t* __restrict__ v,
     const bf16_t* __restrict__ o, const bf16_t* __restrict__ dout, const float* __restrict__ lse,
@@ -722,7 +742,7 @@
     int* linb_s = row_s + NK;
     int* rid_s = linb_s + NK;
     float* tab_s = reinterpret_cast<float*>(rid_s + NK);
-    int* flag_s = reinterpret_cast<int*>(tab_s + G.tls);
+    int* flag_s = reinterpret_cast<int*>(tab_s + (IMG ? 0 : G.tls));
     bf16_t* T_s = reinterpret_cast<bf16_t*>(flag_s + 4);
 
     const int tid = threadIdx.x, lane = tid & 63, wave = tid >> 6, lg = lane >> 4, lr = lane & 15;
@@ -731,12 +751,22 @@
     const int N = G.g.N;
     constexpr int nt = NKT;
     const bool tb = bias != nullptr;
-    if (tid == 0) *flag_s = 0;
+    if (!IMG && tid == 0) *flag_s = 0;
     token_rows<NK>(G, grp, row_s, tid, NTHR);
     if (wave == 0) { ONE_T(0); }
 
     Frag8 kf[2], vf[2];
     float kmv[2];
+    const f32x4_t* imb = nullptr;
+    f32x4_t im[2][2];
+    if (IMG && wave < NWC) {
+        const int pc = rid ? rid[grp % G.nW] : 0;
+        imb = reinterpret_cast<const f32x4_t*>(bias) + ((int64_t)(pc * G.g.nH + h) * IMG_TILES(NKT) + NKT * NKT) * 64 + lane;
+#pragma unroll
+        for (int half = 0; half < 2; ++half)
+#pragma unroll
+            for (int ti = 0; ti < 2; ++ti) im[half][ti] = imb[((wave * 2 + ti) * NKT + half) * 64];
+    }
     if (wave < NWC) {
 #pragma unroll
         for (int ti = 0; ti < 2; ++ti) {
@@ -773,12 +803,12 @@
         static_assert(NK <= NTHR, "one token per thread");
         const int wloc = grp % G.nW;
         const float lv = (tid < N) ? lse[((int64_t)grp * G.g.nH + h) * N + tid] : 0.f;
-        const int rv = (rid && tid < N) ? rid[wloc * N + tid] : 0, rv0 = rid ? rid[wloc * N] : 0;
+        const int rv = (!IMG && rid && tid < N) ? rid[wloc * N + tid] : 0, rv0 = (!IMG && rid) ? rid[wloc * N] : 0;
         float tv[NTAB];
 #pragma unroll
         for (int j = 0; j < NTAB; ++j) {
             const int i = tid + j * NTHR;
-            tv[j] = i < G.tbn ? bias[(int64_t)(G.tb0 + i) * G.g.nH + h] : 0.f;
+            tv[j] = (!IMG && i < G.tbn) ? bias[(int64_t)(G.tb0 + i) * G.g.nH + h] : 0.f;
         }
 #pragma unroll
         for (int j = 0; j < NP; ++j) {
@@ -799,8 +829,8 @@
         }
         if (tid < NK) {
             L_s[tid] = (tid < N) ? -lv * LOG2E : -INFINITY;
-            linb_s[tid] = (tid < N) ? 4 * win_lin(G, tid) : 0;
-            if (rid) {
+            if (!IMG) linb_s[tid] = (tid < N) ? 4 * win_lin(G, tid) : 0;
+            if (!IMG && rid) {
                 rid_s[tid] = rv;
                 if (tid < N && rv != rv0) *flag_s = 1;
             }
@@ -808,7 +838,7 @@
 #pragma unroll
         for (int j = 0; j < NTAB; ++j) {
             const int i = tid + j * NTHR;
-            if (i < G.tbn) tab_s[i] = tv[j] * LOG2E;
+            if (!IMG && i < G.tbn) tab_s[i] = tv[j] * LOG2E;
         }
     }
     if (wave == 0) { ONE_T(1); }
@@ -892,10 +922,10 @@
             dkacc[ti][c] = (f32x4_t){0.f, 0.f, 0.f, 0.f};
         }
         const int nk = (wave * 2 + ti) * 16 + lr;
-        rk[ti] = (rid && nk < N) ? rid_s[nk] : 0;
-        ko[ti] = linb_s[nk < N ? nk : 0] - 4 * G.tcst;
-    }
-    const bool masked = rid && *flag_s != 0;
+        rk[ti] = (!IMG && rid && nk < N) ? rid_s[nk] : 0;
+        ko[ti] = IMG ? 0 : linb_s[nk < N ? nk : 0] - 4 * G.tcst;
+    }
+    const bool masked = IMG ? false : (rid && *flag_s != 0);
 
     auto chunk = [&](int p, auto nh_c, auto masked_c) {
         constexpr int NH = decltype(nh_c)::value;
@@ -915,13 +945,16 @@
             const float4 L4 = *reinterpret_cast<const float4*>(L_s + qn0);
             const float4 D4 = *reinterpret_cast<const float4*>(D_s + qn0);
             const float Lr[4] = {L4.x, L4.y, L4.z, L4.w}, Dr[4] = {D4.x, D4.y, D4.z, D4.w};
-            const int4 qb = *reinterpret_cast<const int4*>(linb_s + qn0);
+            int4 qb = make_int4(0, 0, 0, 0);
+            if (!IMG) qb = *reinterpret_cast<const int4*>(linb_s + qn0);
             int4 rq4 = make_int4(0, 0, 0, 0);
             if (MASKED) rq4 = *reinterpret_cast<const int4*>(rid_s + qn0);
 #pragma unroll
             for (int ti = 0; ti < 2; ++ti) {
                 f32x4_t sacc, pacc = {0.f, 0.f, 0.f, 0.f};
-                if (!(ONE_ABL & 16)) {
+                if (IMG) {
+                    sacc = im[half][ti];
+                } else if (!(ONE_ABL & 16)) {
                     const char* tp = reinterpret_cast<const char*>(tab_s) - ko[ti];
                     sacc[0] = kmv[ti] + *reinterpret_cast<const float*>(tp + qb.x);
                     sacc[1] = kmv[ti] + *reinterpret_cast<const float*>(tp + qb.y);
@@ -951,6 +984,14 @@
                 if (!(ONE_ABL & 4))
                 *reinterpret_cast<uint2*>(Tw + (half * 2 + ti) * 256 + lr * 16 + lg * 4) =
                     make_uint2(dsf[ti].u[half * 2 + 0], dsf[ti].u[half * 2 + 1]);
+            }
+        }
+        if (IMG) {
+#pragma unroll
+            for (int half = 0; half < 2; ++half) {
+                const int qtn = min(2 * p + 2 + half, NKT - 1);
+#pragma unroll
+                for (int ti = 0; ti < 2; ++ti) im[half][ti] = imb[((wave * 2 + ti) * NKT + qtn) * 64];
             }
         }
 #pragma unroll
@@ -1172,6 +1213,63 @@
         const float t = wave_sum(a[hh]);
         if (lane == 0) static_cast<float*>(en.dtable)[slot * en.nH + h0 + hh] += t;
     }
+}
+
+struct ImgEntry {
+    const float* table;
+    float* img;
+    const int* rid;
+    const int* pmap;
+    int N, nH, nkt, nW, npat, hw, bww, ts_d, ts_h, toff, block_begin, tiles;
+};
+struct ImgTable {
+    ImgEntry e[CLV_ATTN_IMG_MAX];
+    int n;
+};
+__global__ void __launch_bounds__(256) attn_img_build_kernel(ImgTable tab) {
+    int idx = 0;
+    for (int i = 1; i < tab.n; ++i)
+        if ((int)blockIdx.x >= tab.e[i].block_begin) idx = i;
+    const ImgEntry& en = tab.e[idx];
+    const int nkt = en.nkt, tiles = IMG_TILES(nkt), bpp = (en.tiles * 64 + 255) / 256;
+    const int lb = (int)blockIdx.x - en.block_begin, ch = lb / bpp, c = ch / en.nH, h = ch - c * en.nH;
+    constexpr int MAXN = 256;
+    __shared__ int wrep, lin_s[MAXN], rid_s[MAXN];
+    if (threadIdx.x == 0) wrep = 0x7fffffff;
+    __syncthreads();
+    if (c > 0 && en.rid && en.pmap)
+        for (int w = threadIdx.x; w < en.nW; w += 256)
+            if (en.pmap[w] == c) atomicMin(&wrep, w);
+    __syncthreads();
+    const int* rr = (c > 0 && en.rid && en.pmap && wrep < en.nW) ? en.rid + (int64_t)wrep * en.N : nullptr;
+    for (int n = threadIdx.x; n < MAXN; n += 256) {
+        const int m = n < en.N ? n : 0;
+        const int tz = m / en.hw, tr = m - tz * en.hw;
+        const int ty = tr / en.bww, tx = tr - ty * en.bww;
+        lin_s[n] = tz * en.ts_d + ty * en.ts_h + tx;
+        rid_s[n] = rr ? rr[m] : 0;
+    }
+    __syncthreads();
+    const int i = (lb - ch * bpp) * 256 + (int)threadIdx.x;
+    if (c >= en.npat || i >= en.tiles * 64) return;
+    const int lane = i & 63, tile = i >> 6, lg = lane >> 4, lr = lane & 15;
+    const bool fwd = tile < nkt * nkt;
+    const int tl = fwd ? tile : tile - nkt * nkt;
+    const int qt = fwd ? tl / nkt : tl % nkt, kt = fwd ? tl % nkt : tl / nkt;
+    float out[4];
+#pragma unroll
+    for (int r = 0; r < 4; ++r) {
+        const int q = qt * 16 + (fwd ? lr : lg * 4 + r), k = kt * 16 + (fwd ? lg * 4 + r : lr);
+        float v = 0.f;
+        if (q < en.N) {
+            const int kc = k < en.N ? k : 0;
+            const float t = __fmul_rn(en.table[(int64_t)(lin_s[q] - lin_s[kc] + en.toff) * en.nH + h], LOG2E);
+            v = fwd ? (k < en.N ? t : -INFINITY) : __fadd_rn(k < en.N ? 0.f : -INFINITY, t);
+            if (rr) v = __fadd_rn(v, rid_s[kc] != rid_s[q] ? -100.0f * LOG2E : 0.0f);
+        }
+        out[r] = v;
+    }
+    reinterpret_cast<float4*>(en.img)[((int64_t)ch * tiles + tile) * 64 + lane] = make_float4(out[0], out[1], out[2], out[3]);
 }
 
 constexpr int F32_MAXT = 16;
@@ -1545,18 +1643,35 @@
     CLV_ATTR((attn_bwd_dkv_kernel<HD, NKE, false, 0>));
     CLV_ATTR((attn_bwd_dkv_kernel<HD, NKE, true, 0>));
     if constexpr (HD == 32 && (NKT == 13 || NKT == 25)) CLV_ATTR((attn_bwd_one_kernel<HD, NKT>));
+    if constexpr (IMG_SHAPE(HD, NKT)) {
+        CLV_ATTR((attn_fwd_kernel<HD, NKT, false, 1, true>));
+        CLV_ATTR((attn_bwd_one_kernel<HD, NKT, true>));
+    }
 #undef CLV_ATTR
+}
+
+template <int HD, int NKT>
+bool img_ok(const Geom& G) {
+    return IMG_SHAPE(HD, NKT) && G.g.mode == 1 && G.nparts == 1 && !G.drop_thresh && G.tlen > 0 && (G.g.N + 15) / 16 == NKT;
 }
 
 template <int HD, int NKT>
 int launch_fwd(const void* q, const void* k, const void* v, void* o, float* lse, const float* bias,
-               const int32_t* rid, const float* kmask, const unsigned long long* seed, const Geom& G, hipStream_t st) {
+               const int32_t* rid, const float* kmask, const unsigned long long* seed, const Geom& G, hipStream_t st,
+               const float* img = nullptr, const int32_t* pmap = nullptr) {
     const int bl = bias ? G.tls : 0;
     const size_t lds = fwd_lds<HD, NKT>(bl, G.g.mode == 1);
     if (lds > MAX_LDS || dq_lds<HD, NKT>(bl) > MAX_LDS || dkv_lds<HD, NKT>(bl) > MAX_LDS) return CLV_ERR_UNSUPPORTED;
     if (G.g.mode == 1 && G.drop_thresh) return CLV_ERR_UNSUPPORTED;
     set_attrs<HD, NKT>();
     const int nblk = G.g.groups * G.g.nH * G.tsplit * G.nparts;
+    if constexpr (IMG_SHAPE(HD, NKT)) {
+        if (img && bias && img_ok<HD, NKT>(G)) {
+            attn_fwd_kernel<HD, NKT, false, 1, true><<<dim3(nblk), dim3(THREADS), fwd_lds<HD, NKT>(0, true), st>>>(
+                (const bf16_t*)q, (const bf16_t*)k, (const bf16_t*)v, (bf16_t*)o, lse, img, pmap, nullptr, seed, G);
+            return clv_check_launch();
+        }
+    }
     if (G.nparts == 1) {
         CLV_PICK(attn_fwd_kernel, <<<dim3(nblk), dim3(THREADS), lds, st>>>((const bf16_t*)q, (const bf16_t*)k,
                  (const bf16_t*)v, (bf16_t*)o, lse, bias, rid, kmask, seed, G));
@@ -1594,7 +1709,7 @@
 int launch_bwd(const void* q, const void* k, const void* v, const void* o, const void* dout,
                const float* lse, const float* bias, const int32_t* rid, const float* kmask, void* dq,
                void* dk, void* dv, float* dbias, float* dsum, void* work, const unsigned long long* seed, int stages,
-               const Geom& G, hipStream_t st) {
+               const Geom& G, hipStream_t st, const float* img = nullptr, const int32_t* pmap = nullptr) {
     const int bl = bias ? G.tls : 0;
     constexpr int NKE = (NKT + 1) & ~1;
     const size_t lds_a = dq_lds<HD, NKT>(bl), lds_b = dkv_lds<HD, NKE>(bl);
@@ -1618,6 +1733,14 @@
     }
     const bool one = one_eligible<HD, NKT>(G, bias != nullptr) && (stages & 5) == 5;
     auto launch_one = [&](const Geom& Gx, int groups) {
+        if constexpr (IMG_SHAPE(HD, NKT)) {
+            if (img && img_ok<HD, NKT>(G)) {
+                attn_bwd_one_kernel<HD, NKT, true><<<dim3(groups * G.g.nH), dim3((ONE_CWAVES(NKT) + ONE_SWAVES(NKT)) * 64), one_lds<HD, NKT>(0), st>>>(
+                    (const bf16_t*)q, (const bf16_t*)k, (const bf16_t*)v, (const bf16_t*)o, (const bf16_t*)dout, lse, img, pmap,
+                    dq_out, dk_out, dv_out, (bf16_t*)work, dsum, Gx);
+                return;
+            }
+        }
         if constexpr (HD == 32 && (NKT == 13 || NKT == 25))
             attn_bwd_one_kernel<HD, NKT><<<dim3(groups * G.g.nH), dim3((ONE_CWAVES(NKT) + ONE_SWAVES(NKT)) * 64), one_lds<HD, NKT>(bl), st>>>(
                 (const bf16_t*)q, (const bf16_t*)k, (const bf16_t*)v, (const bf16_t*)o, (const bf16_t*)dout, lse, bias, rid,
@@ -1714,11 +1837,12 @@
         default: return CLV_ERR_UNSUPPORTED;                         \
     }
 
-}
-
-extern "C" int clv_attn_fwd(const void* q, const void* k, const void* v, void* o, float* lse,
-                            const float* bias, const int32_t* rid, const float* kmask, const void* seed,
-                            const ClvAttnGeom* geom, void* stream) {
+template <int HD, int NKT>
+int query_img(const Geom& G) { return img_ok<HD, NKT>(G) ? 1 : 0; }
+
+int attn_fwd_any(const void* q, const void* k, const void* v, void* o, float* lse, const float* bias, const int32_t* rid,
+                 const float* kmask, const void* seed, const ClvAttnGeom* geom, void* stream, const float* img,
+                 const int32_t* pmap) {
     Geom G;
     if (!q || !k || !v || !o || !lse || !make_geom(geom, G)) return CLV_ERR_ARG;
     if (G.drop_thresh && !seed) return CLV_ERR_ARG;
@@ -1727,9 +1851,78 @@
     if (rid && G.g.mode != 1) return CLV_ERR_ARG;
     const int nkt = pick_nkt(G.nparts > 1 ? G.pt16 : G.g.N);
     hipStream_t st = (hipStream_t)stream;
+    if (img && rid && !pmap) return CLV_ERR_ARG;
     if (G.g.hd == 16) { DISPATCH_NKT(16, launch_fwd, q, k, v, o, lse, bias, rid, kmask, sp, G, st) }
-    if (G.g.hd == 32) { DISPATCH_NKT(32, launch_fwd, q, k, v, o, lse, bias, rid, kmask, sp, G, st) }
+    if (G.g.hd == 32) { DISPATCH_NKT(32, launch_fwd, q, k, v, o, lse, bias, rid, kmask, sp, G, st, img, pmap) }
     DISPATCH_NKT(64, launch_fwd, q, k, v, o, lse, bias, rid, kmask, sp, G, st)
+}
+
+}
+
+extern "C" int clv_attn_fwd(const void* q, const void* k, const void* v, void* o, float* lse,
+                            const float* bias, const int32_t* rid, const float* kmask, const void* seed,
+                            const ClvAttnGeom* geom, void* stream) {
+    return attn_fwd_any(q, k, v, o, lse, bias, rid, kmask, seed, geom, stream, nullptr, nullptr);
+}
+
+extern "C" int clv_attn_fwd_img(const void* q, const void* k, const void* v, void* o, float* lse, const float* bias,
+                                const int32_t* rid, const float* img, const int32_t* pmap, const ClvAttnGeom* geom,
+                                void* stream) {
+    return attn_fwd_any(q, k, v, o, lse, bias, rid, nullptr, nullptr, geom, stream, img, pmap);
+}
+
+extern "C" int clv_attn_img_supported(const ClvAttnGeom* geom) {
+    Geom G;
+    if (!make_geom(geom, G) || G.g.hd != 32) return 0;
+    const int nkt = pick_nkt(G.g.N);
+    const int r = [&]() -> int { DISPATCH_NKT(32, query_img, G) }();
+    return r == 1 ? 1 : 0;
+}
+
+extern "C" int clv_attn_img_wins(const ClvAttnGeom* geom) {
+    Geom G;
+    if (!clv_attn_img_supported(geom) || !make_geom(geom, G)) return 0;
+    return (G.tsplit == 1 && G.g.groups >= 128) ? 1 : 0;
+}
+
+extern "C" int64_t clv_attn_img_floats(const ClvAttnGeom* geom, int32_t npat) {
+    if (npat <= 0 || !clv_attn_img_supported(geom)) return 0;
+    return (int64_t)npat * geom->nH * IMG_TILES(pick_nkt(geom->N)) * 256;
+}
+
+extern "C" int clv_attn_img_build_batch(const ClvAttnImgEntry* entries, int32_t n, void* stream) {
+    if (!entries || n <= 0 || n > CLV_ATTN_IMG_MAX) return CLV_ERR_ARG;
+    ImgTable tab;
+    int blocks = 0;
+    for (int i = 0; i < n; ++i) {
+        const ClvAttnImgEntry& src = entries[i];
+        Geom G;
+        if (!src.table || !src.img || src.npat <= 0 || !clv_attn_img_supported(src.geom) || !make_geom(src.geom, G))
+            return CLV_ERR_ARG;
+        if (src.npat > 1 && (!src.rid || !src.pmap)) return CLV_ERR_ARG;
+        if (reinterpret_cast<uintptr_t>(src.img) & 15) return CLV_ERR_ARG;
+        ImgEntry& en = tab.e[i];
+        en.table = src.table;
+        en.img = src.img;
+        en.rid = src.rid;
+        en.pmap = src.pmap;
+        en.N = G.g.N;
+        en.nH = G.g.nH;
+        en.nkt = pick_nkt(G.g.N);
+        en.nW = G.nW;
+        en.npat = src.npat;
+        en.hw = G.g.bwh * G.g.bww;
+        en.bww = G.g.bww;
+        en.ts_d = G.ts_d;
+        en.ts_h = G.ts_h;
+        en.toff = G.tcst + G.tb0;
+        en.block_begin = blocks;
+        en.tiles = src.fwd_only ? en.nkt * en.nkt : IMG_TILES(en.nkt);
+        blocks += src.npat * G.g.nH * ((en.tiles * 64 + 255) / 256);
+    }
+    tab.n = n;
+    hipLaunchKernelGGL(attn_img_build_kernel, dim3((unsigned)blocks), dim3(256), 0, (hipStream_t)stream, tab);
+    return clv_check_launch();
 }
 
 extern "C" int64_t clv_attn_bwd_work_bytes(const ClvAttnGeom* geom) {
@@ -1786,10 +1979,11 @@
     return clv_check_launch();
 }
 
-extern "C" int clv_attn_bwd(const void* q, const void* k, const void* v, const void* o, const void* dout,
-                            const float* lse, const float* bias, const int32_t* rid, const float* kmask,
-                            void* dq, void* dk, void* dv, float* dbias, float* dsum, void* work,
-                            const void* seed, int32_t stages, const ClvAttnGeom* geom, void* stream) {
+static int attn_bwd_any(const void* q, const void* k, const void* v, const void* o, const void* dout,
+                        const float* lse, const float* bias, const int32_t* rid, const float* kmask,
+                        void* dq, void* dk, void* dv, float* dbias, float* dsum, void* work,
+                        const void* seed, int32_t stages, const ClvAttnGeom* geom, void* stream, const float* img,
+                        const int32_t* pmap) {
     Geom G;
     const unsigned long long* sp = (const unsigned long long*)seed;
     if (stages == 0) stages = 7;
@@ -1800,8 +1994,25 @@
     const int nkt = pick_nkt(G.nparts > 1 ? G.pt16 : G.g.N);
     hipStream_t st = (hipStream_t)stream;
     if (G.g.hd == 16) { DISPATCH_NKT(16, launch_bwd, q, k, v, o, dout, lse, bias, rid, kmask, dq, dk, dv, dbias, dsum, work, sp, stages, G, st) }
-    if (G.g.hd == 32) { DISPATCH_NKT(32, launch_bwd, q, k, v, o, dout, lse, bias, rid, kmask, dq, dk, dv, dbias, dsum, work, sp, stages, G, st) }
+    if (img && rid && !pmap) return CLV_ERR_ARG;
+    if (G.g.hd == 32) { DISPATCH_NKT(32, launch_bwd, q, k, v, o, dout, lse, bias, rid, kmask, dq, dk, dv, dbias, dsum, work, sp, stages, G, st, img, pmap) }
     DISPATCH_NKT(64, launch_bwd, q, k, v, o, dout, lse, bias, rid, kmask, dq, dk, dv, dbias, dsum, work, sp, stages, G, st)
+}
+
+extern "C" int clv_attn_bwd(const void* q, const void* k, const void* v, const void* o, const void* dout,
+                            const float* lse, const float* bias, const int32_t* rid, const float* kmask,
+                            void* dq, void* dk, void* dv, float* dbias, float* dsum, void* work,
+                            const void* seed, int32_t stages, const ClvAttnGeom* geom, void* stream) {
+    return attn_bwd_any(q, k, v, o, dout, lse, bias, rid, kmask, dq, dk, dv, dbias, dsum, work, seed, stages, geom, stream,
+                        nullptr, nullptr);
+}
+
+extern "C" int clv_attn_bwd_img(const void* q, const void* k, const void* v, const void* o, const void* dout,
+                                const float* lse, const float* bias, const int32_t* rid, const float* img,
+                                const int32_t* pmap, void* dq, void* dk, void* dv, float* dbias, float* dsum, void* work,
+                                int32_t stages, const ClvAttnGeom* geom, void* stream) {
+    return attn_bwd_any(q, k, v, o, dout, lse, bias, rid, nullptr, dq, dk, dv, dbias, dsum, work, nullptr, stages, geom, stream,
+                        img, pmap);
 }
 
 
diff --git a/clover_amd/ops.py b/clover_amd/ops.py
--- a/clover_amd/ops.py
+++ b/clover_amd/ops.py
@@ -1423,7 +1423,7 @@
 class _Attention(torch.autograd.Function):
 
     @staticmethod
-    def forward(ctx, qkv, table, rid, kmask, geom_kw, seed):
+    def forward(ctx, qkv, table, rid, kmask, geom_kw, seed, img=None):
         _need_gpu(qkv)
         assert qkv.dtype == BF16 and qkv.is_contiguous()
         g = ClvAttnGeom(**geom_kw)
@@ -1442,11 +1442,19 @@
         seq_work = torch.empty(wbytes, device=qkv.device, dtype=torch.uint8) if wbytes > 0 else None
         g.work = seq_work.data_ptr() if seq_work is not None else None
         base = qkv.data_ptr()
+        if img is not None and (tab is None or kmask is not None or seed is not None):
+            img = None
         with _Timed(_kname('attn_fwd_kernel', g), *_attn_work(g, False)):
-            check(_lib.lib().clv_attn_fwd(C.c_void_p(base), C.c_void_p(base + 2 * Cdim),
-                                          C.c_void_p(base + 4 * Cdim), _ptr(o), _ptr(lse), _ptr(tab), _ptr(rid),
-                                          _ptr(kmask), _ptr(seed), C.byref(g), _stream()), 'clv_attn_fwd')
+            if img is not None:
+                check(_lib.lib().clv_attn_fwd_img(C.c_void_p(base), C.c_void_p(base + 2 * Cdim),
+                                                  C.c_void_p(base + 4 * Cdim), _ptr(o), _ptr(lse), _ptr(tab), _ptr(rid),
+                                                  _ptr(img[0]), _ptr(img[1]), C.byref(g), _stream()), 'clv_attn_fwd_img')
+            else:
+                check(_lib.lib().clv_attn_fwd(C.c_void_p(base), C.c_void_p(base + 2 * Cdim),
+                                              C.c_void_p(base + 4 * Cdim), _ptr(o), _ptr(lse), _ptr(tab), _ptr(rid),
+                                              _ptr(kmask), _ptr(seed), C.byref(g), _stream()), 'clv_attn_fwd')
         ctx.save_for_backward(qkv, o, lse, tab, rid, kmask, seed)
+        ctx.img = img if img is not None and img[2] else None
         ctx.geom = g
         ctx.tref = table
         return o
@@ -1475,49 +1483,76 @@
         args = (C.c_void_p(b), C.c_void_p(b + 2 * Cdim), C.c_void_p(b + 4 * Cdim), _ptr(o), _ptr(doc), _ptr(lse),
                 _ptr(tab), _ptr(rid), _ptr(kmask), C.c_void_p(d), C.c_void_p(d + 2 * Cdim),
                 C.c_void_p(d + 4 * Cdim), _ptr(dtab), _ptr(dsum), _ptr(work), _ptr(seed))
+        img = ctx.img
+
+        def bwd(stages):
+            if img is not None:
+                check(L.clv_attn_bwd_img(*args[:8], _ptr(img[0]), _ptr(img[1]), *args[9:15], stages, C.byref(g), _stream()),
+                      'clv_attn_bwd_img')
+            else:
+                check(L.clv_attn_bwd(*args, stages, C.byref(g), _stream()), 'clv_attn_bwd')
         if PROF is None and SEGMENT is not None and sink is not None:
             part = torch.empty(L.clv_attn_dbias_partial_bytes(C.byref(g)), device=qkv.device, dtype=torch.uint8)
             g.work = part.data_ptr()
-            check(L.clv_attn_bwd(*args, 15, C.byref(g), _stream()), 'clv_attn_bwd')
+            bwd(15)
             ent = _lib.ClvDbiasGather()
             check(L.clv_attn_dbias_gather_entry(C.byref(g), _ptr(work), _ptr(dtab), C.byref(ent)), 'clv_attn_dbias_gather_entry')
             g.work = None
             SEGMENT.dbias.append(DbiasItem(ent, part, dtab, g.dbias_index))
         elif PROF is None:
-            check(L.clv_attn_bwd(*args, 0, C.byref(g), _stream()), 'clv_attn_bwd')
+            bwd(0)
         elif tab is not None and L.clv_attn_bwd_one_kernel(C.byref(g)) == 1:
             fl, by = _attn_work(g, True)
             with _Timed(f'attn_bwd_one_kernel<{g.hd}, {(g.N + 15) // 16}>', fl, by):
-                check(L.clv_attn_bwd(*args, 5, C.byref(g), _stream()), 'clv_attn_bwd')
-            check(L.clv_attn_bwd(*args, 2, C.byref(g), _stream()), 'clv_attn_bwd')
+                bwd(5)
+            bwd(2)
         else:
             fl, by = _attn_work(g, True)
             with _Timed(_kname('attn_bwd_dq_kernel', g), fl * 0.4, by * 0.5):
-                check(L.clv_attn_bwd(*args, 1, C.byref(g), _stream()), 'clv_attn_bwd')
-            check(L.clv_attn_bwd(*args, 2, C.byref(g), _stream()), 'clv_attn_bwd')
+                bwd(1)
+            bwd(2)
             with _Timed(_kname('attn_bwd_dkv_kernel', g), fl * 0.6, by * 0.5):
-                check(L.clv_attn_bwd(*args, 4, C.byref(g), _stream()), 'clv_attn_bwd')
+                bwd(4)
         if sink is not None:
             _delivered(ctx.tref)
             dtab = None
         elif dtab is not None:
             dtab = dtab.to(ctx.tref.dtype)
-        return dqkv, dtab, None, None, None, None
-
-
-def window_attention(qkv, table, rid, window, shift, num_heads, table_window=None):
-    B, D, H, W, C3 = qkv.shape
-    Cdim = C3 // 3
+        return dqkv, dtab, None, None, None, None, None
+
+
+class AttnImage:
+    __slots__ = ('img', 'pmap', 'key', 'backward')
+
+    def __init__(self, img, pmap, key, backward=True):
+        self.img, self.pmap, self.key, self.backward = img, pmap, key, backward
+
+
+def attn_image_key(kw):
+    return tuple(kw[k] for k in ('groups', 'N', 'nH', 'hd', 'D', 'H', 'W', 'wd', 'wh', 'ww', 'sd', 'sh', 'sw',
+                                 'bwd', 'bwh', 'bww'))
+
+
+def window_attention_kw(B, D, H, W, Cdim, window, shift, num_heads, table_window):
     hd = Cdim // num_heads
     N = window[0] * window[1] * window[2]
     nW = (D // window[0]) * (H // window[1]) * (W // window[2])
-    tw = tuple(table_window or window) if table is not None else (0, 0, 0)
-    kw = dict(mode=1, groups=B * nW, N=N, nH=num_heads, hd=hd, D=D, H=H, W=W, wd=window[0], wh=window[1],
-              ww=window[2], sd=shift[0], sh=shift[1], sw=shift[2], bwd=tw[0], bwh=tw[1], bww=tw[2],
-              scale=float(hd) ** -0.5)
+    tw = tuple(table_window) if table_window is not None else (0, 0, 0)
+    return dict(mode=1, groups=B * nW, N=N, nH=num_heads, hd=hd, D=D, H=H, W=W, wd=window[0], wh=window[1],
+                ww=window[2], sd=shift[0], sh=shift[1], sw=shift[2], bwd=tw[0], bwh=tw[1], bww=tw[2],
+                scale=float(hd) ** -0.5)
+
+
+def window_attention(qkv, table, rid, window, shift, num_heads, table_window=None, image=None):
+    B, D, H, W, C3 = qkv.shape
+    kw = window_attention_kw(B, D, H, W, C3 // 3, window, shift, num_heads,
+                             tuple(table_window or window) if table is not None else None)
     if parity.enabled():
         return parity.attention(qkv, table, rid, None, kw)
-    return _Attention.apply(qkv, table, rid, None, kw, None)
+    img = None
+    if image is not None and table is not None and image.key == attn_image_key(kw) and (rid is None) == (image.pmap is None):
+        img = (image.img, image.pmap, image.backward)
+    return _Attention.apply(qkv, table, rid, None, kw, None, img)
 
 
 _DROPOUT_COUNTER = {}
@@ -1631,7 +1666,7 @@
         return _LongSeqAttention.apply(qkv, kmask, num_heads, float(dropout_p), seed)
     kw = dict(mode=0, groups=B, N=S, nH=num_heads, hd=hd, scale=float(hd) ** -0.5, dropout_p=float(dropout_p))
     seed = next_dropout_seed(qkv.device) if dropout_p > 0 else None
-    return _Attention.apply(qkv, None, None, kmask, kw, seed)
+    return _Attention.apply(qkv, None, None, kmask, kw, seed, None)
 
 
 class _PatchEmbed(torch.autograd.Function):
diff --git a/include/clover_hip.h b/include/clover_hip.h
--- a/include/clover_hip.h
+++ b/include/clover_hip.h
@@ -57,6 +57,27 @@
 int clv_attn_dbias_gather_entry(const ClvAttnGeom* geom_host, void* work, float* dbias, ClvDbiasGather* out);
 int64_t clv_attn_dbias_partial_bytes(const ClvAttnGeom* geom_host);
 int clv_attn_dbias_gather_batch(const ClvDbiasGather* entries, int32_t n, void* stream);
+
+#define CLV_ATTN_IMG_MAX 16
+typedef struct ClvAttnImgEntry {
+    const ClvAttnGeom* geom;
+    const float* table;
+    const int32_t* rid;
+    const int32_t* pmap;
+    float* img;
+    int32_t npat;
+    int32_t fwd_only;
+} ClvAttnImgEntry;
+int clv_attn_img_supported(const ClvAttnGeom* geom_host);
+int clv_attn_img_wins(const ClvAttnGeom* geom_host);
+int64_t clv_attn_img_floats(const ClvAttnGeom* geom_host, int32_t npat);
+int clv_attn_img_build_batch(const ClvAttnImgEntry* entries, int32_t n, void* stream);
+int clv_attn_fwd_img(const void* q, const void* k, const void* v, void* o, float* lse, const float* bias,
+                     const int32_t* rid, const float* img, const int32_t* pmap, const ClvAttnGeom* geom_host, void* stream);
+int clv_attn_bwd_img(const void* q, const void* k, const void* v, const void* o, const void* dout,
+                     const float* lse, const float* bias, const int32_t* rid, const float* img, const int32_t* pmap,
+                     void* dq, void* dk, void* dv, float* dbias, float* dsum, void* work,
+                     int32_t stages, const ClvAttnGeom* geom_host, void* stream);
 
 int clv_softmax_rows_fwd(const void* scores, const float* kmask, void* p, void* pd, const void* seed, int64_t rows,
                          int32_t S, int32_t ld, int32_t rows_per_group, float scale, float dropout_p, void* stream);
```

New measurement: 756.8 pairs/s. No clear change (-0.2%).
